# alibaba/EasyParallelLibrary

Measured on AMD Instinct MI355X. Metric: samples_per_sec, higher is better.
Workload: dtype bf16; 1 GPU; model=bert-large, global_batch=128, seq_len=512, parallelism=dp1

## Files before the change

csrc/bindings.hip:

```cpp

#include <hip/hip_runtime.h>
#include <torch/extension.h>
#include <ATen/hip/impl/HIPStreamMasqueradingAsCUDA.h>

#include <cstdint>

#include "kernels/attn_block_order.h"

namespace epl {
void register_comm(py::module& m);
}

extern "C" {
void epl_fused_adamw(float*, unsigned short*, const void*, bool, float*,
                     float*, int64_t, float, float, float, float, float, int,
                     float, hipStream_t);
void epl_lamb_phase1(const float*, const void*, bool, float*, float*, float*,
                     const int*, float*, float*, int64_t, float, float, float,
                     float, int, float, hipStream_t);
void epl_lamb_phase2(float*, unsigned short*, const float*, const int*,
                     const float*, int64_t, float, hipStream_t);
void epl_layer_norm_fwd(void*, const void*, const void*, void*, const void*,
                        const void*, float*, float*, int64_t, int64_t, float,
                        bool, hipStream_t);
void epl_layer_norm_bwd(void*, float*, float*, const void*, const void*,
                        const void*, const float*, const float*, float*,
                        float*, int64_t, int64_t, int64_t, bool,
                        hipStream_t);
void epl_layer_norm_bwd_fused(void*, float*, float*, float*, const void*,
                              const void*, const void*, const void*,
                              const float*, const float*, float*, float*,
                              float*, int64_t, int64_t, int64_t, bool,
                              hipStream_t);
void epl_bias_gelu_fwd(void*, const void*, const void*, int64_t, int64_t,
                       bool, hipStream_t);
void epl_bias_gelu_bwd(void*, float*, const void*, const void*, const void*,
                       float*, int64_t, int64_t, int64_t, bool,
                       hipStream_t);
void epl_ce_rowstats(const void*, const int64_t*, float*, float*, float*,
                     int64_t, int64_t, int64_t, int64_t, bool, hipStream_t);
void epl_ce_backward(void*, const void*, const int64_t*, const float*,
                     const float*, const float*, int64_t, int64_t, int64_t,
                     int64_t, float, bool, hipStream_t);
void epl_scale(void*, int64_t, float, bool, hipStream_t);
void epl_f32_to_bf16(unsigned short*, const float*, int64_t, hipStream_t);
void epl_bf16_to_f32(float*, const unsigned short*, int64_t, hipStream_t);
void epl_sqnorm(const void*, int64_t, float*, bool, hipStream_t);
void epl_colsum(void*, const void*, float*, int64_t, int64_t, int64_t,
                bool, hipStream_t);
void run_mfma_probe(const unsigned short*, const unsigned short*, float*,
                    hipStream_t);
void run_tr_read_probe(short*, short*, int, hipStream_t);
void run_block_order_probe(int*, int, int, hipStream_t);
void epl_moe_dispatch_fwd(void*, const void*, const int64_t*,
                          const int64_t*, const int64_t*, int64_t, int64_t,
                          int64_t, hipStream_t);
void epl_moe_dispatch_bwd(void*, const void*, const int64_t*,
                          const int64_t*, const int64_t*, int64_t, int64_t,
                          int64_t, int64_t, hipStream_t);
void epl_moe_combine_fwd(void*, const void*, const float*, const int64_t*,
                         const int64_t*, const int64_t*, int64_t, int64_t,
                         int64_t, int64_t, hipStream_t);
void epl_moe_combine_bwd(void*, float*, const void*, const void*,
                         const float*, const int64_t*, const int64_t*,
                         const int64_t*, int64_t, int64_t, int64_t,
                         hipStream_t);
int64_t epl_moe_router_waves(int64_t, int64_t);
void epl_moe_router_fwd(const void*, int64_t*, float*, float*, int64_t*,
                        float*, float*, float*, int*, int64_t, int64_t,
                        int64_t, bool, bool, hipStream_t);
void epl_moe_router_bwd(void*, const void*, const float*, const int64_t*,
                        const float*, const int64_t*, const float*,
                        const float*, int64_t, int64_t, int64_t, bool, bool,
                        hipStream_t);
void epl_attn_fwd(const void*, const void*, const void*, void*, float*,
                  int64_t, int64_t, float, bool, int64_t, int64_t,
                  const int64_t*,
                  const int64_t*, unsigned int*, int64_t,
                  unsigned long long, int, float, const int*, hipStream_t);
void epl_attn_bwd(const void*, const void*, const void*, const void*,
                  const void*, const float*, float*, void*, void*, void*,
                  int64_t, int64_t, float, bool, int64_t, const int64_t*,
                  const int64_t*, const int64_t*, const int64_t*, int,
                  const unsigned int*, int64_t, float, int64_t,
                  const float*, const int*, hipStream_t);
void epl_rms_norm_fwd(void*, const void*, const void*, void*, const void*,
                      float*, int64_t, int64_t, float, hipStream_t);
int64_t epl_rms_norm_bwd_parts(int64_t, int64_t);
void epl_rms_norm_bwd(void*, float*, const void*, const void*, const void*,
                      const float*, const void*, float*, int64_t, int64_t,
                      hipStream_t);
void epl_rope(void*, const float*, const float*, int64_t, int64_t, int64_t,
              int64_t, int64_t, int64_t, int64_t, int64_t, bool,
              hipStream_t);
void epl_swiglu_fwd(void*, const void*, int64_t, int64_t, hipStream_t);
void epl_swiglu_bwd(void*, const void*, const void*, int64_t, int64_t,
                    hipStream_t);
}

namespace {

hipStream_t cur_stream() {
  return c10::hip::getCurrentHIPStreamMasqueradingAsCUDA().stream();
}

void check(const at::Tensor& t, at::ScalarType dtype, const char* name) {
  TORCH_CHECK(t.is_cuda(), name, " must be a device tensor");
  TORCH_CHECK(t.is_contiguous(), name, " must be contiguous");
  TORCH_CHECK(t.scalar_type() == dtype, name, " has dtype ", t.scalar_type(),
              ", expected ", dtype);
}

void check_arena(const at::Tensor& t, const char* name) {
  TORCH_CHECK(t.is_cuda(), name, " must be a device tensor");
  TORCH_CHECK(t.is_contiguous(), name, " must be contiguous");
}

void check_aligned(const at::Tensor& t, size_t bytes, const char* name) {
  TORCH_CHECK(reinterpret_cast<uintptr_t>(t.data_ptr()) % bytes == 0, name,
              " must start on a ", bytes, "-byte boundary");
}

bool is_bf16(const at::Tensor& t) {
  TORCH_CHECK(t.scalar_type() == at::kBFloat16 || t.scalar_type() == at::kFloat,
              "expected bf16 or fp32, got ", t.scalar_type());
  return t.scalar_type() == at::kBFloat16;
}

void fused_adamw(at::Tensor master, c10::optional<at::Tensor> param_bf16,
                 at::Tensor grad, at::Tensor m, at::Tensor v, double lr,
                 double beta1, double beta2, double eps, double weight_decay,
                 int64_t step, double inv_scale) {
  check(master, at::kFloat, "master");
  check(m, at::kFloat, "m");
  check(v, at::kFloat, "v");
  check_arena(grad, "grad");
  const bool gbf = is_bf16(grad);
  unsigned short* pb = nullptr;
  if (param_bf16.has_value()) {
    check(*param_bf16, at::kBFloat16, "param_bf16");
    TORCH_CHECK(param_bf16->numel() == master.numel(),
                "arena size mismatch");
    check_aligned(*param_bf16, 16, "param_bf16");
    pb = reinterpret_cast<unsigned short*>(param_bf16->data_ptr());
  }
  const int64_t n = master.numel();
  TORCH_CHECK(grad.numel() == n && m.numel() == n && v.numel() == n,
              "arena size mismatch");
  check_aligned(master, 32, "master");
  check_aligned(m, 32, "m");
  check_aligned(v, 32, "v");
  check_aligned(grad, gbf ? 16 : 32, "grad");
  epl_fused_adamw(master.data_ptr<float>(), pb, grad.data_ptr(), gbf,
                  m.data_ptr<float>(), v.data_ptr<float>(), n, (float)lr,
                  (float)beta1, (float)beta2, (float)eps, (float)weight_decay,
                  (int)step, (float)inv_scale, cur_stream());
}

void lamb_phase1(at::Tensor master, at::Tensor grad, at::Tensor m,
                 at::Tensor v, at::Tensor update, at::Tensor chunk_of,
                 at::Tensor wnorm_sq, at::Tensor unorm_sq, double beta1,
                 double beta2, double eps, double weight_decay, int64_t step,
                 double inv_scale) {
  check(master, at::kFloat, "master");
  check(update, at::kFloat, "update");
  check(chunk_of, at::kInt, "chunk_of");
  const bool gbf = is_bf16(grad);
  epl_lamb_phase1(master.data_ptr<float>(), grad.data_ptr(), gbf,
                  m.data_ptr<float>(), v.data_ptr<float>(),
                  update.data_ptr<float>(), chunk_of.data_ptr<int>(),
                  wnorm_sq.data_ptr<float>(), unorm_sq.data_ptr<float>(),
                  master.numel(), (float)beta1, (float)beta2, (float)eps,
                  (float)weight_decay, (int)step, (float)inv_scale,
                  cur_stream());
}

void lamb_phase2(at::Tensor master, c10::optional<at::Tensor> param_bf16,
                 at::Tensor update, at::Tensor chunk_of, at::Tensor ratio,
                 double lr) {
  check(master, at::kFloat, "master");
  unsigned short* pb = nullptr;
  if (param_bf16.has_value())
    pb = reinterpret_cast<unsigned short*>(param_bf16->data_ptr());
  epl_lamb_phase2(master.data_ptr<float>(), pb, update.data_ptr<float>(),
                  chunk_of.data_ptr<int>(), ratio.data_ptr<float>(),
                  master.numel(), (float)lr, cur_stream());
}

void layer_norm_fwd(at::Tensor out, at::Tensor x,
                    c10::optional<at::Tensor> res,
                    c10::optional<at::Tensor> sum_out, at::Tensor gamma,
                    at::Tensor beta, at::Tensor mean, at::Tensor rstd,
                    double eps) {
  const bool bf16 = is_bf16(x);
  const int64_t cols = x.size(-1);
  const int64_t rows = x.numel() / cols;
  TORCH_CHECK(!bf16 || cols % 8 == 0, "bf16 LayerNorm needs cols % 8 == 0");
  check(mean, at::kFloat, "mean");
  check(rstd, at::kFloat, "rstd");
  const void* res_p = nullptr;
  void* sum_p = nullptr;
  if (res.has_value()) {
    TORCH_CHECK(sum_out.has_value(),
                "fused residual LayerNorm needs sum_out");
    TORCH_CHECK(res->numel() == x.numel() && sum_out->numel() == x.numel());
    res_p = res->data_ptr();
    sum_p = sum_out->data_ptr();
  }
  epl_layer_norm_fwd(out.data_ptr(), x.data_ptr(), res_p, sum_p,
                     gamma.data_ptr(), beta.data_ptr(),
                     mean.data_ptr<float>(), rstd.data_ptr<float>(), rows,
                     cols, (float)eps, bf16, cur_stream());
}

void layer_norm_bwd(at::Tensor dx, at::Tensor dgamma, at::Tensor dbeta,
                    at::Tensor dy, at::Tensor x, at::Tensor gamma,
                    at::Tensor mean, at::Tensor rstd) {
  const bool bf16 = is_bf16(x);
  const int64_t cols = x.size(-1);
  const int64_t rows = x.numel() / cols;
  TORCH_CHECK(!bf16 || cols % 8 == 0, "bf16 LayerNorm needs cols % 8 == 0");
  TORCH_CHECK((size_t)cols * 2 * sizeof(float) <= 128 * 1024,
              "LayerNorm backward supports cols <= 16384");
  check(dgamma, at::kFloat, "dgamma");
  check(dbeta, at::kFloat, "dbeta");
  float* dgp = nullptr;
  float* dbp = nullptr;
  at::Tensor ws;
  const bool fast = bf16 && cols % 8 == 0 && cols <= 2048;
  int64_t nparts = 0;
  if (fast) {
    const int64_t wave_rows = (rows + 3) / 4;
    nparts = (wave_rows < 1024 ? wave_rows : 1024) * 4;
    ws = at::empty({2, nparts, cols}, dgamma.options());
    dgp = ws.data_ptr<float>();
    dbp = dgp + nparts * cols;
  }
  epl_layer_norm_bwd(dx.data_ptr(), dgamma.data_ptr<float>(),
                     dbeta.data_ptr<float>(), dy.data_ptr(), x.data_ptr(),
                     gamma.data_ptr(), mean.data_ptr<float>(),
                     rstd.data_ptr<float>(), dgp, dbp, nparts, rows, cols,
                     bf16, cur_stream());
}

void layer_norm_bwd_fused(at::Tensor dx, at::Tensor dgamma, at::Tensor dbeta,
                          at::Tensor dy, at::Tensor x, at::Tensor gamma,
                          at::Tensor mean, at::Tensor rstd,
                          c10::optional<at::Tensor> dadd,
                          c10::optional<at::Tensor> colsum_out) {
  const bool bf16 = is_bf16(x);
  const int64_t cols = x.size(-1);
  const int64_t rows = x.numel() / cols;
  TORCH_CHECK(!bf16 || cols % 8 == 0, "bf16 LayerNorm needs cols % 8 == 0");
  TORCH_CHECK((size_t)cols * 2 * sizeof(float) <= 128 * 1024,
              "LayerNorm backward supports cols <= 16384");
  check(dgamma, at::kFloat, "dgamma");
  check(dbeta, at::kFloat, "dbeta");
  TORCH_CHECK(dx.numel() == x.numel() && dy.numel() == x.numel());
  TORCH_CHECK(dgamma.numel() == cols && dbeta.numel() == cols);
  const bool fast = bf16 && cols % 8 == 0 && cols <= 2048;
  const bool fused = dadd.has_value() || colsum_out.has_value();
  TORCH_CHECK(fast || !fused,
              "layer_norm_bwd_fused: dadd/colsum_out need the bf16 fast "
              "path (cols % 8 == 0, cols <= 2048)");
  const void* dadd_p = nullptr;
  float* cs_out = nullptr;
  if (dadd.has_value()) {
    check(*dadd, x.scalar_type(), "dadd");
    TORCH_CHECK(dadd->numel() == x.numel(), "dadd shape mismatch");
    dadd_p = dadd->data_ptr();
  }
  if (colsum_out.has_value()) {
    check(*colsum_out, at::kFloat, "colsum_out");
    TORCH_CHECK(colsum_out->numel() == cols, "colsum_out shape mismatch");
    cs_out = colsum_out->data_ptr<float>();
  }
  float* dgp = nullptr;
  float* dbp = nullptr;
  float* csp = nullptr;
  at::Tensor ws;
  int64_t nparts = 0;
  if (fast) {
    const int64_t wave_rows = (rows + 3) / 4;
    nparts = (wave_rows < 1024 ? wave_rows : 1024) * 4;
    ws = at::empty({cs_out ? 3 : 2, nparts, cols}, dgamma.options());
    dgp = ws.data_ptr<float>();
    dbp = dgp + nparts * cols;
    if (cs_out) csp = dbp + nparts * cols;
  }
  epl_layer_norm_bwd_fused(dx.data_ptr(), dgamma.data_ptr<float>(),
                           dbeta.data_ptr<float>(), cs_out, dy.data_ptr(),
                           x.data_ptr(), gamma.data_ptr(), dadd_p,
                           mean.data_ptr<float>(), rstd.data_ptr<float>(),
                           dgp, dbp, csp, nparts, rows, cols, bf16,
                           cur_stream());
}

void bias_gelu_fwd(at::Tensor out, at::Tensor x, at::Tensor bias) {
  const bool bf16 = is_bf16(x);
  const int64_t cols = x.size(-1);
  const int64_t rows = x.numel() / cols;
  TORCH_CHECK(!bf16 || cols % 8 == 0, "bf16 bias_gelu needs cols % 8 == 0");
  epl_bias_gelu_fwd(out.data_ptr(), x.data_ptr(), bias.data_ptr(), rows, cols,
                    bf16, cur_stream());
}

void bias_gelu_bwd(at::Tensor dx, at::Tensor dbias, at::Tensor dy,
                   at::Tensor x, at::Tensor bias) {
  const bool bf16 = is_bf16(x);
  const int64_t cols = x.size(-1);
  const int64_t rows = x.numel() / cols;
  TORCH_CHECK(!bf16 || cols % 8 == 0, "bf16 bias_gelu needs cols % 8 == 0");
  TORCH_CHECK((size_t)cols * sizeof(float) <= 128 * 1024,
              "bias_gelu backward supports cols <= 32768");
  check(dbias, at::kFloat, "dbias");
  float* dbp = nullptr;
  int64_t nwaves = 0;
  at::Tensor ws;
  if (bf16 && cols % 512 == 0) {
    const int64_t segs = cols / 512;
    int64_t per_seg = rows < 1024 ? rows : 1024;
    per_seg = (per_seg + 3) / 4 * 4;
    nwaves = segs * per_seg;
    ws = at::empty({nwaves, 512}, dbias.options());
    dbp = ws.data_ptr<float>();
  }
  epl_bias_gelu_bwd(dx.data_ptr(), dbias.data_ptr<float>(), dy.data_ptr(),
                    x.data_ptr(), bias.data_ptr(), dbp, nwaves, rows, cols,
                    bf16, cur_stream());
}

void ce_rowstats(at::Tensor logits, at::Tensor targets, at::Tensor row_max,
                 at::Tensor row_sumexp, at::Tensor target_logit,
                 int64_t vocab_begin, int64_t ignore_index) {
  const bool bf16 = is_bf16(logits);
  const int64_t cols = logits.size(-1);
  const int64_t rows = logits.numel() / cols;
  check(targets, at::kLong, "targets");
  epl_ce_rowstats(logits.data_ptr(), targets.data_ptr<int64_t>(),
                  row_max.data_ptr<float>(), row_sumexp.data_ptr<float>(),
                  target_logit.data_ptr<float>(), rows, cols, vocab_begin,
                  ignore_index, bf16, cur_stream());
}

void ce_backward(at::Tensor dlogits, at::Tensor logits, at::Tensor targets,
                 at::Tensor gmax, at::Tensor gsumexp, at::Tensor dloss,
                 int64_t vocab_begin, int64_t ignore_index, double scale) {
  const bool bf16 = is_bf16(logits);
  const int64_t cols = logits.size(-1);
  const int64_t rows = logits.numel() / cols;
  epl_ce_backward(dlogits.data_ptr(), logits.data_ptr(),
                  targets.data_ptr<int64_t>(), gmax.data_ptr<float>(),
                  gsumexp.data_ptr<float>(), dloss.data_ptr<float>(), rows,
                  cols, vocab_begin, ignore_index, (float)scale, bf16,
                  cur_stream());
}

void scale_(at::Tensor t, double s) {
  check_arena(t, "t");
  const bool bf16 = is_bf16(t);
  check_aligned(t, 16, "t");
  epl_scale(t.data_ptr(), t.numel(), (float)s, bf16, cur_stream());
}

void f32_to_bf16(at::Tensor dst, at::Tensor src) {
  check(dst, at::kBFloat16, "dst");
  check(src, at::kFloat, "src");
  TORCH_CHECK(dst.numel() == src.numel());
  check_aligned(dst, 16, "dst");
  check_aligned(src, 16, "src");
  epl_f32_to_bf16(reinterpret_cast<unsigned short*>(dst.data_ptr()),
                  src.data_ptr<float>(), src.numel(), cur_stream());
}

void bf16_to_f32(at::Tensor dst, at::Tensor src) {
  check(dst, at::kFloat, "dst");
  check(src, at::kBFloat16, "src");
  TORCH_CHECK(dst.numel() == src.numel());
  check_aligned(dst, 16, "dst");
  check_aligned(src, 16, "src");
  epl_bf16_to_f32(dst.data_ptr<float>(),
                  reinterpret_cast<unsigned short*>(src.data_ptr()),
                  src.numel(), cur_stream());
}

static void attn_strides(const at::Tensor& t, int64_t* out3,
                         const char* name) {
  TORCH_CHECK(t.dim() == 4 && (t.size(3) == 64 || t.size(3) == 128), name,
              " must be [B,H,S,64|128]");
  TORCH_CHECK(t.stride(3) == 1, name, " last dim must be contiguous");
  TORCH_CHECK(t.stride(2) % 8 == 0 && t.stride(1) % 8 == 0,
              name, " row strides must be 16-byte aligned");
  out3[0] = t.stride(0);
  out3[1] = t.stride(1);
  out3[2] = t.stride(2);
}

static void attn_check_grid(int64_t bh, int64_t seq, bool causal) {
  const int64_t nqb = (seq + 127) / 128;
  TORCH_CHECK(nqb <= 65535, "attention: seq ", seq, " needs ", nqb,
              " 128-row blocks, more than the 65535 a launch can hold");
  TORCH_CHECK(causal || bh <= 65535, "attention: non-causal batch*heads ",
              bh, " exceeds the 65535 blocks of gridDim.y");
}

static const int* attn_seqlens(const c10::optional<at::Tensor>& seqlens,
                               const at::Tensor& q) {
  if (!seqlens.has_value()) return nullptr;
  check(*seqlens, at::kInt, "seqlens");
  TORCH_CHECK(seqlens->numel() == q.size(0), "seqlens must hold ",
              q.size(0), " lengths (one per sample), got ",
              seqlens->numel());
  TORCH_CHECK(seqlens->device() == q.device(),
              "seqlens must be on the device of q");
  return seqlens->data_ptr<int>();
}

void attn_fwd(at::Tensor q, at::Tensor k, at::Tensor v, at::Tensor out,
              at::Tensor lse, double scale, bool causal,
              c10::optional<at::Tensor> drop_mask, int64_t seed,
              int64_t drop_thresh, double inv_keep,
              c10::optional<at::Tensor> seqlens) {
  TORCH_CHECK(q.is_cuda() && q.scalar_type() == at::kBFloat16);
  int64_t in_s[3], o_s[3], tmp[3];
  attn_strides(q, in_s, "q");
  attn_strides(k, tmp, "k");
  TORCH_CHECK(tmp[0] == in_s[0] && tmp[1] == in_s[1] && tmp[2] == in_s[2],
              "q/k/v must share strides");
  attn_strides(v, tmp, "v");
  TORCH_CHECK(tmp[0] == in_s[0] && tmp[1] == in_s[1] && tmp[2] == in_s[2],
              "q/k/v must share strides");
  attn_strides(out, o_s, "out");
  check(lse, at::kFloat, "lse");
  const int64_t heads = q.size(1);
  const int64_t seq = q.size(2);
  const int64_t head_dim = q.size(3);
  const int64_t bh = q.size(0) * heads;
  attn_check_grid(bh, seq, causal);
  unsigned int* mptr = nullptr;
  int64_t mask_w = (seq + 31) / 32;
  if (drop_mask.has_value()) {
    check(*drop_mask, at::kInt, "drop_mask");
    TORCH_CHECK(drop_mask->numel() == bh * seq * mask_w,
                "drop_mask size mismatch");
    TORCH_CHECK(drop_thresh > 0 && drop_thresh < 256, "drop_thresh range");
    mptr = reinterpret_cast<unsigned int*>(drop_mask->data_ptr());
  }
  epl_attn_fwd(q.data_ptr(), k.data_ptr(), v.data_ptr(), out.data_ptr(),
               lse.data_ptr<float>(), bh, seq, (float)scale, causal, heads,
               head_dim, in_s, o_s, mptr, mask_w,
               (unsigned long long)seed, (int)drop_thresh,
               (float)inv_keep, attn_seqlens(seqlens, q), cur_stream());
}

void attn_bwd(at::Tensor q, at::Tensor k, at::Tensor v, at::Tensor out,
              at::Tensor dout, at::Tensor lse, at::Tensor delta_ws,
              at::Tensor dq, at::Tensor dk, at::Tensor dv, double scale,
              bool causal, bool split_dkdv,
              c10::optional<at::Tensor> drop_mask, double inv_keep,
              c10::optional<at::Tensor> dlse,
              c10::optional<at::Tensor> seqlens) {
  int64_t in_s[3], o_s[3], do_s[3], g_s[3], tmp[3];
  attn_strides(q, in_s, "q");
  attn_strides(out, o_s, "out");
  attn_strides(dout, do_s, "dout");
  attn_strides(dq, g_s, "dq");
  attn_strides(dk, tmp, "dk");
  TORCH_CHECK(tmp[0] == g_s[0] && tmp[1] == g_s[1] && tmp[2] == g_s[2],
              "dq/dk/dv must share strides");
  attn_strides(dv, tmp, "dv");
  TORCH_CHECK(tmp[0] == g_s[0] && tmp[1] == g_s[1] && tmp[2] == g_s[2],
              "dq/dk/dv must share strides");
  const int64_t heads = q.size(1);
  const int64_t seq = q.size(2);
  const int64_t bh = q.size(0) * heads;
  attn_check_grid(bh, seq, causal);
  check(delta_ws, at::kFloat, "delta_ws");
  const unsigned int* mptr = nullptr;
  int64_t mask_w = (seq + 31) / 32;
  if (drop_mask.has_value()) {
    check(*drop_mask, at::kInt, "drop_mask");
    mptr = reinterpret_cast<const unsigned int*>(drop_mask->data_ptr());
  }
  const float* dlse_ptr = nullptr;
  if (dlse.has_value()) {
    check(*dlse, at::kFloat, "dlse");
    TORCH_CHECK(dlse->numel() == bh * seq, "dlse size mismatch");
    dlse_ptr = dlse->data_ptr<float>();
  }
  epl_attn_bwd(q.data_ptr(), k.data_ptr(), v.data_ptr(), out.data_ptr(),
               dout.data_ptr(), lse.data_ptr<float>(),
               delta_ws.data_ptr<float>(), dq.data_ptr(), dk.data_ptr(),
               dv.data_ptr(), bh, seq, (float)scale, causal, heads, in_s,
               o_s, do_s, g_s, split_dkdv ? 1 : 0, mptr, mask_w,
               (float)inv_keep, q.size(3), dlse_ptr,
               attn_seqlens(seqlens, q), cur_stream());
}

void tr_read_probe(at::Tensor out_gather, at::Tensor out_tr,
                   int64_t head_dim) {
  TORCH_CHECK(head_dim == 64 || head_dim == 128, "head_dim must be 64|128");
  check(out_gather, at::kShort, "out_gather");
  check(out_tr, at::kShort, "out_tr");
  const int64_t n = 4 * (head_dim / 32) * 64 * 8;
  TORCH_CHECK(out_gather.numel() == n && out_tr.numel() == n,
              "probe outputs must hold ", n, " elements");
  run_tr_read_probe(reinterpret_cast<short*>(out_gather.data_ptr()),
                    reinterpret_cast<short*>(out_tr.data_ptr()),
                    (int)head_dim, cur_stream());
}

void attn_block_order_probe(at::Tensor out, int64_t n, int64_t bh) {
  check(out, at::kInt, "out");
  TORCH_CHECK(n >= 1 && n <= 65535 && bh >= 1 && bh <= 65535,
              "grid dimensions must lie in [1, 65535]");
  TORCH_CHECK(out.numel() == 2 * n * bh, "out must hold ", 2 * n * bh,
              " elements");
  run_block_order_probe(out.data_ptr<int>(), (int)n, (int)bh, cur_stream());
}

at::Tensor attn_block_order_host(int64_t n, int64_t bh) {
  TORCH_CHECK(n >= 1 && n <= 65535 && bh >= 1 && bh <= 65535,
              "grid dimensions must lie in [1, 65535]");
  at::Tensor out = at::empty({n * bh, 2}, at::kInt);
  int* p = out.data_ptr<int>();
  for (int64_t y = 0; y < bh; ++y)
    for (int64_t x = 0; x < n; ++x) {
      const attn_order::Block b = attn_order::block_of(
          (unsigned)x, (unsigned)y, (unsigned)n, (unsigned)bh);
      p[2 * (x + n * y)] = (int)b.bh;
      p[2 * (x + n * y) + 1] = (int)b.blk;
    }
  return out;
}

void mfma_probe(at::Tensor A, at::Tensor B, at::Tensor D) {
  check(A, at::kBFloat16, "A");
  check(B, at::kBFloat16, "B");
  check(D, at::kFloat, "D");
  run_mfma_probe(reinterpret_cast<const unsigned short*>(A.data_ptr()),
                 reinterpret_cast<const unsigned short*>(B.data_ptr()),
                 D.data_ptr<float>(), cur_stream());
}

static void check_idx(const at::Tensor& t, const char* name) {
  TORCH_CHECK(t.is_cuda() && t.is_contiguous() &&
              t.scalar_type() == at::kLong, name,
              " must be a contiguous int64 device tensor");
}

void moe_dispatch_fwd(at::Tensor disp, at::Tensor x, at::Tensor fe,
                      at::Tensor pos, at::Tensor ft, int64_t cap) {
  check(disp, at::kBFloat16, "disp");
  check(x, at::kBFloat16, "x");
  check_idx(fe, "fe"); check_idx(pos, "pos"); check_idx(ft, "ft");
  const int64_t hidden = x.size(-1);
  TORCH_CHECK(hidden % 8 == 0, "hidden % 8");
  epl_moe_dispatch_fwd(disp.data_ptr(), x.data_ptr(),
                       fe.data_ptr<int64_t>(), pos.data_ptr<int64_t>(),
                       ft.data_ptr<int64_t>(), fe.numel(), hidden, cap,
                       cur_stream());
}

void moe_dispatch_bwd(at::Tensor dx, at::Tensor ddisp, at::Tensor fe,
                      at::Tensor pos, at::Tensor inv, int64_t k,
                      int64_t cap) {
  check(dx, at::kBFloat16, "dx");
  check(ddisp, at::kBFloat16, "ddisp");
  check_idx(fe, "fe"); check_idx(pos, "pos"); check_idx(inv, "inv");
  const int64_t hidden = dx.size(-1);
  epl_moe_dispatch_bwd(dx.data_ptr(), ddisp.data_ptr(),
                       fe.data_ptr<int64_t>(), pos.data_ptr<int64_t>(),
                       inv.data_ptr<int64_t>(), dx.numel() / hidden, k,
                       hidden, cap, cur_stream());
}

void moe_combine_fwd(at::Tensor out, at::Tensor h, at::Tensor fw,
                     at::Tensor fe, at::Tensor pos, at::Tensor inv,
                     int64_t k, int64_t cap) {
  check(out, at::kBFloat16, "out");
  check(h, at::kBFloat16, "h");
  check(fw, at::kFloat, "fw");
  check_idx(fe, "fe"); check_idx(pos, "pos"); check_idx(inv, "inv");
  const int64_t hidden = out.size(-1);
  epl_moe_combine_fwd(out.data_ptr(), h.data_ptr(), fw.data_ptr<float>(),
                      fe.data_ptr<int64_t>(), pos.data_ptr<int64_t>(),
                      inv.data_ptr<int64_t>(), out.numel() / hidden, k,
                      hidden, cap, cur_stream());
}

void moe_combine_bwd(at::Tensor dh, at::Tensor dfw, at::Tensor dout,
                     at::Tensor h, at::Tensor fw, at::Tensor fe,
                     at::Tensor pos, at::Tensor ft, int64_t cap) {
  check(dh, at::kBFloat16, "dh");
  check(dout, at::kBFloat16, "dout");
  check(h, at::kBFloat16, "h");
  check(fw, at::kFloat, "fw");
  check(dfw, at::kFloat, "dfw");
  check_idx(fe, "fe"); check_idx(pos, "pos"); check_idx(ft, "ft");
  const int64_t hidden = dh.size(-1);
  epl_moe_combine_bwd(dh.data_ptr(), dfw.data_ptr<float>(),
                      dout.data_ptr(), h.data_ptr(), fw.data_ptr<float>(),
                      fe.data_ptr<int64_t>(), pos.data_ptr<int64_t>(),
                      ft.data_ptr<int64_t>(), fe.numel(), hidden, cap,
                      cur_stream());
}

static bool aligned16(const at::Tensor& t) {
  return reinterpret_cast<uintptr_t>(t.data_ptr()) % 16 == 0;
}

static void router_extents(const at::Tensor& logits, int64_t k, int64_t* n,
                           int64_t* e) {
  TORCH_CHECK(logits.is_cuda() && logits.is_contiguous() &&
              logits.dim() == 2,
              "logits must be a contiguous 2-D device tensor");
  *n = logits.size(0);
  *e = logits.size(1);
  TORCH_CHECK(k == 1 || k == 2, "moe router: k must be 1 or 2, got ", k);
  TORCH_CHECK(*e >= 2 && *e <= 256,
              "moe router: 2 <= num_experts <= 256, got ", *e);
  TORCH_CHECK(*n >= 1 && *n < (int64_t(1) << 30),
              "moe router: 1 <= tokens < 2^30, got ", *n);
}

void moe_router_fwd(at::Tensor logits, int64_t k, at::Tensor topi,
                    at::Tensor topw, at::Tensor lse, at::Tensor counts,
                    at::Tensor psum, at::Tensor losses) {
  const bool bf16 = is_bf16(logits);
  int64_t n, e;
  router_extents(logits, k, &n, &e);
  check_idx(topi, "topi");
  check(topw, at::kFloat, "topw");
  check(lse, at::kFloat, "lse");
  check_idx(counts, "counts");
  check(psum, at::kFloat, "psum");
  check(losses, at::kFloat, "losses");
  TORCH_CHECK(topi.numel() == n * k && topw.numel() == n * k,
              "topi / topw must hold tokens * k elements");
  TORCH_CHECK(lse.numel() == n, "lse must hold one element per token");
  TORCH_CHECK(counts.numel() == e && psum.numel() == e,
              "counts / psum must hold one element per expert");
  TORCH_CHECK(losses.numel() == 2, "losses must hold 2 elements");
  const int64_t waves = epl_moe_router_waves(n, e);
  at::Tensor p_part = at::empty({waves * e + waves},
                                logits.options().dtype(at::kFloat));
  at::Tensor c_part = at::empty({waves * e},
                                logits.options().dtype(at::kInt));
  epl_moe_router_fwd(logits.data_ptr(), topi.data_ptr<int64_t>(),
                     topw.data_ptr<float>(), lse.data_ptr<float>(),
                     counts.data_ptr<int64_t>(), psum.data_ptr<float>(),
                     losses.data_ptr<float>(), p_part.data_ptr<float>(),
                     c_part.data_ptr<int>(), n, e, k, bf16,
                     aligned16(logits), cur_stream());
}

void moe_router_bwd(at::Tensor dlogits, at::Tensor logits, at::Tensor lse,
                    at::Tensor topi, at::Tensor dw, at::Tensor counts,
                    at::Tensor g_bal, at::Tensor g_z, int64_t k) {
  const bool bf16 = is_bf16(logits);
  int64_t n, e;
  router_extents(logits, k, &n, &e);
  check(dlogits, logits.scalar_type(), "dlogits");
  TORCH_CHECK(dlogits.numel() == n * e, "dlogits must match logits");
  check(lse, at::kFloat, "lse");
  check_idx(topi, "topi");
  check(dw, at::kFloat, "dw");
  check_idx(counts, "counts");
  check(g_bal, at::kFloat, "g_bal");
  check(g_z, at::kFloat, "g_z");
  TORCH_CHECK(lse.numel() == n, "lse must hold one element per token");
  TORCH_CHECK(topi.numel() == n * k && dw.numel() == n * k,
              "topi / dw must hold tokens * k elements");
  TORCH_CHECK(counts.numel() == e,
              "counts must hold one element per expert");
  TORCH_CHECK(g_bal.numel() == 1 && g_z.numel() == 1,
              "g_bal / g_z must hold one element");
  epl_moe_router_bwd(dlogits.data_ptr(), logits.data_ptr(),
                     lse.data_ptr<float>(), topi.data_ptr<int64_t>(),
                     dw.data_ptr<float>(), counts.data_ptr<int64_t>(),
                     g_bal.data_ptr<float>(), g_z.data_ptr<float>(), n, e, k,
                     bf16, aligned16(logits) && aligned16(dlogits),
                     cur_stream());
}

void colsum(at::Tensor dy, at::Tensor db, at::Tensor partial) {
  const bool bf16 = is_bf16(dy);
  TORCH_CHECK(dy.is_cuda() && dy.is_contiguous() && dy.dim() == 2,
              "dy must be a contiguous 2-D device tensor");
  const int64_t rows = dy.size(0), cols = dy.size(1);
  TORCH_CHECK(cols % 8 == 0, "cols must be a multiple of 8");
  TORCH_CHECK(db.numel() == cols && db.scalar_type() == dy.scalar_type());
  const int64_t stripes = partial.numel() / cols;
  TORCH_CHECK(stripes >= 1 && partial.scalar_type() == at::kFloat);
  epl_colsum(db.data_ptr(), dy.data_ptr(), partial.data_ptr<float>(), rows,
             cols, stripes, bf16, cur_stream());
}

void sqnorm(at::Tensor t, at::Tensor out) {
  check_arena(t, "t");
  const bool bf16 = is_bf16(t);
  check(out, at::kFloat, "out");
  TORCH_CHECK(out.numel() >= 1, "out must hold one element");
  epl_sqnorm(t.data_ptr(), t.numel(), out.data_ptr<float>(), bf16,
             cur_stream());
}


static void check_llama_bf16(const at::Tensor& t, const at::Device& dev,
                             const char* name) {
  check(t, at::kBFloat16, name);
  TORCH_CHECK(t.device() == dev, name, " is on another device");
  TORCH_CHECK(aligned16(t), name, " must be 16-byte aligned");
}

static void check_llama_f32(const at::Tensor& t, const at::Device& dev,
                            int64_t numel, const char* name) {
  check(t, at::kFloat, name);
  TORCH_CHECK(t.device() == dev, name, " is on another device");
  TORCH_CHECK(aligned16(t), name, " must be 16-byte aligned");
  TORCH_CHECK(t.numel() == numel, name, " must hold ", numel, " elements");
}

static void rms_extents(const at::Tensor& x, int64_t* rows, int64_t* cols) {
  TORCH_CHECK(x.dim() >= 1 && x.numel() > 0, "rms_norm: empty input");
  *cols = x.size(-1);
  *rows = x.numel() / *cols;
  TORCH_CHECK(*cols % 8 == 0 && *cols >= 8 && *cols <= 8192,
              "rms_norm: native widths are multiples of 8 up to 8192, got ",
              *cols);
}

void rms_norm_fwd(at::Tensor out, at::Tensor x, c10::optional<at::Tensor> res,
                  c10::optional<at::Tensor> s_out, at::Tensor gamma,
                  at::Tensor rstd, double eps) {
  int64_t rows, cols;
  const at::Device dev = x.device();
  check_llama_bf16(x, dev, "x");
  rms_extents(x, &rows, &cols);
  check_llama_bf16(out, dev, "out");
  check_llama_bf16(gamma, dev, "gamma");
  TORCH_CHECK(out.numel() == x.numel(), "out must match x");
  TORCH_CHECK(gamma.numel() == cols, "gamma must hold cols elements");
  check_llama_f32(rstd, dev, rows, "rstd");
  TORCH_CHECK(res.has_value() == s_out.has_value(),
              "rms_norm_fwd: res and s come together");
  const void* res_p = nullptr;
  void* s_p = nullptr;
  if (res.has_value()) {
    check_llama_bf16(*res, dev, "res");
    check_llama_bf16(*s_out, dev, "s");
    TORCH_CHECK(res->numel() == x.numel() && s_out->numel() == x.numel(),
                "res and s must match x");
    res_p = res->data_ptr();
    s_p = s_out->data_ptr();
  }
  epl_rms_norm_fwd(out.data_ptr(), x.data_ptr(), res_p, s_p,
                   gamma.data_ptr(), rstd.data_ptr<float>(), rows, cols,
                   (float)eps, cur_stream());
}

void rms_norm_bwd(at::Tensor dx, at::Tensor dgamma, at::Tensor dy,
                  at::Tensor s, at::Tensor gamma, at::Tensor rstd,
                  c10::optional<at::Tensor> dadd) {
  int64_t rows, cols;
  const at::Device dev = s.device();
  check_llama_bf16(s, dev, "s");
  rms_extents(s, &rows, &cols);
  check_llama_bf16(dx, dev, "dx");
  check_llama_bf16(dy, dev, "dy");
  check_llama_bf16(gamma, dev, "gamma");
  TORCH_CHECK(dx.numel() == s.numel() && dy.numel() == s.numel(),
              "dx and dy must match s");
  TORCH_CHECK(gamma.numel() == cols, "gamma must hold cols elements");
  check_llama_f32(dgamma, dev, cols, "dgamma");
  check_llama_f32(rstd, dev, rows, "rstd");
  const void* dadd_p = nullptr;
  if (dadd.has_value()) {
    check_llama_bf16(*dadd, dev, "dadd");
    TORCH_CHECK(dadd->numel() == s.numel(), "dadd must match s");
    dadd_p = dadd->data_ptr();
  }
  const int64_t nparts = epl_rms_norm_bwd_parts(rows, cols);
  at::Tensor ws = at::empty({nparts, cols}, dgamma.options());
  epl_rms_norm_bwd(dx.data_ptr(), dgamma.data_ptr<float>(), dy.data_ptr(),
                   s.data_ptr(), gamma.data_ptr(), rstd.data_ptr<float>(),
                   dadd_p, ws.data_ptr<float>(), rows, cols, cur_stream());
}

void rope_(at::Tensor x, at::Tensor cos_t, at::Tensor sin_t, int64_t pos0,
           bool inverse) {
  TORCH_CHECK(x.is_cuda() && x.scalar_type() == at::kBFloat16,
              "rope_: x must be a bf16 device tensor");
  TORCH_CHECK(x.dim() == 4, "rope_: x must be a [B, S, N, D] view");
  const int64_t b = x.size(0), s = x.size(1), n = x.size(2), d = x.size(3);
  TORCH_CHECK(d == 64 || d == 128, "rope_: head_dim must be 64 or 128, got ",
              d);
  TORCH_CHECK(x.stride(3) == 1, "rope_: last dim must be contiguous");
  for (int i = 0; i < 3; ++i)
    TORCH_CHECK(x.size(i) == 1 || (x.stride(i) % 8 == 0 && x.stride(i) >= d),
                "rope_: stride ", i, " must be a multiple of 8 elements "
                "and at least one head, got ", x.stride(i));
  TORCH_CHECK(aligned16(x), "rope_: x must be 16-byte aligned");
  TORCH_CHECK(b * s * n * (d / 16) < (int64_t(1) << 31),
              "rope_: too many elements for one launch");
  const at::Device dev = x.device();
  TORCH_CHECK(cos_t.dim() == 2 && cos_t.size(1) == d / 2,
              "rope_: tables must be [L, D / 2]");
  check_llama_f32(cos_t, dev, cos_t.size(0) * (d / 2), "cos");
  check_llama_f32(sin_t, dev, cos_t.numel(), "sin");
  TORCH_CHECK(pos0 >= 0 && pos0 + s <= cos_t.size(0), "rope_: positions ",
              pos0, " .. ", pos0 + s, " exceed the table length ",
              cos_t.size(0));
  epl_rope(x.data_ptr(), cos_t.data_ptr<float>(), sin_t.data_ptr<float>(),
           x.stride(0), x.stride(1), x.stride(2), b, s, n, d, pos0, inverse,
           cur_stream());
}

static void swiglu_extents(const at::Tensor& gu, int64_t* rows, int64_t* f) {
  TORCH_CHECK(gu.dim() >= 1 && gu.numel() > 0, "swiglu: empty input");
  TORCH_CHECK(gu.size(-1) % 16 == 0, "swiglu: the packed width 2F needs "
              "F % 8 == 0, got ", gu.size(-1));
  *f = gu.size(-1) / 2;
  *rows = gu.numel() / gu.size(-1);
  TORCH_CHECK(*f <= (int64_t(1) << 21), "swiglu: F too large");
}

void swiglu_fwd(at::Tensor out, at::Tensor gu) {
  int64_t rows, f;
  const at::Device dev = gu.device();
  check_llama_bf16(gu, dev, "gu");
  swiglu_extents(gu, &rows, &f);
  check_llama_bf16(out, dev, "out");
  TORCH_CHECK(out.numel() == rows * f, "out must be [rows, F]");
  epl_swiglu_fwd(out.data_ptr(), gu.data_ptr(), rows, f, cur_stream());
}

void swiglu_bwd(at::Tensor dgu, at::Tensor dy, at::Tensor gu) {
  int64_t rows, f;
  const at::Device dev = gu.device();
  check_llama_bf16(gu, dev, "gu");
  swiglu_extents(gu, &rows, &f);
  check_llama_bf16(dgu, dev, "dgu");
  check_llama_bf16(dy, dev, "dy");
  TORCH_CHECK(dgu.numel() == gu.numel(), "dgu must match gu");
  TORCH_CHECK(dy.numel() == rows * f, "dy must be [rows, F]");
  epl_swiglu_bwd(dgu.data_ptr(), dy.data_ptr(), gu.data_ptr(), rows, f,
                 cur_stream());
}

}

PYBIND11_MODULE(TORCH_EXTENSION_NAME, m) {
  m.doc() = "MI355X-native parallel library: RCCL comm core + CDNA4 kernels";
  epl::register_comm(m);
  m.def("fused_adamw", &fused_adamw);
  m.def("colsum", &colsum);
  m.def("lamb_phase1", &lamb_phase1);
  m.def("lamb_phase2", &lamb_phase2);
  m.def("layer_norm_fwd", &layer_norm_fwd);
  m.def("layer_norm_bwd", &layer_norm_bwd);
  m.def("layer_norm_bwd_fused", &layer_norm_bwd_fused, py::arg("dx"),
        py::arg("dgamma"), py::arg("dbeta"), py::arg("dy"), py::arg("x"),
        py::arg("gamma"), py::arg("mean"), py::arg("rstd"),
        py::arg("dadd") = py::none(), py::arg("colsum_out") = py::none());
  m.def("bias_gelu_fwd", &bias_gelu_fwd);
  m.def("bias_gelu_bwd", &bias_gelu_bwd);
  m.def("ce_rowstats", &ce_rowstats);
  m.def("ce_backward", &ce_backward);
  m.def("scale_", &scale_);
  m.def("f32_to_bf16", &f32_to_bf16);
  m.def("bf16_to_f32", &bf16_to_f32);
  m.def("sqnorm", &sqnorm);
  m.def("mfma_probe", &mfma_probe);
  m.def("tr_read_probe", &tr_read_probe);
  m.def("attn_block_order_probe", &attn_block_order_probe);
  m.def("attn_block_order_host", &attn_block_order_host);
  m.def("moe_dispatch_fwd", &moe_dispatch_fwd);
  m.def("moe_dispatch_bwd", &moe_dispatch_bwd);
  m.def("moe_combine_fwd", &moe_combine_fwd);
  m.def("moe_combine_bwd", &moe_combine_bwd);
  m.def("moe_router_fwd", &moe_router_fwd);
  m.def("moe_router_bwd", &moe_router_bwd);
  m.def("moe_router_waves", [](int64_t n, int64_t e) {
    return epl_moe_router_waves(n, e);
  });
  m.def("attn_fwd", &attn_fwd, py::arg("q"), py::arg("k"), py::arg("v"),
        py::arg("out"), py::arg("lse"), py::arg("scale"), py::arg("causal"),
        py::arg("drop_mask"), py::arg("seed"), py::arg("drop_thresh"),
        py::arg("inv_keep"), py::arg("seqlens") = py::none());
  m.def("attn_bwd", &attn_bwd, py::arg("q"), py::arg("k"), py::arg("v"),
        py::arg("out"), py::arg("dout"), py::arg("lse"),
        py::arg("delta_ws"), py::arg("dq"), py::arg("dk"), py::arg("dv"),
        py::arg("scale"), py::arg("causal"), py::arg("split_dkdv"),
        py::arg("drop_mask"), py::arg("inv_keep"), py::arg("dlse"),
        py::arg("seqlens") = py::none());
  m.def("rms_norm_fwd", &rms_norm_fwd, py::arg("out"), py::arg("x"),
        py::arg("res"), py::arg("s"), py::arg("gamma"), py::arg("rstd"),
        py::arg("eps"));
  m.def("rms_norm_bwd", &rms_norm_bwd, py::arg("dx"), py::arg("dgamma"),
        py::arg("dy"), py::arg("s"), py::arg("gamma"), py::arg("rstd"),
        py::arg("dadd") = py::none());
  m.def("rope_", &rope_, py::arg("x"), py::arg("cos"), py::arg("sin"),
        py::arg("pos0"), py::arg("inverse"));
  m.def("swiglu_fwd", &swiglu_fwd);
  m.def("swiglu_bwd", &swiglu_bwd);
}
```

csrc/kernels/kernels.hip:

```cpp

#include <hip/hip_runtime.h>
#include <hip/hip_bf16.h>
#include <cstdint>
#include <cmath>

#define DEV __device__ __forceinline__

namespace {

constexpr int kBlock = 256;
constexpr int kMaxGrid = 4096;

DEV float bf2f(unsigned short u) {
  unsigned int x = (unsigned int)u << 16;
  return __uint_as_float(x);
}

using f32x2 = __attribute__((ext_vector_type(2))) float;
using bf16v2 = __attribute__((ext_vector_type(2))) __bf16;

DEV unsigned int cvt_pk_bf16(float a, float b) {
  f32x2 f = {a, b};
  return __builtin_bit_cast(unsigned int, __builtin_convertvector(f, bf16v2));
}

DEV unsigned short f2bf(float f) {
  return (unsigned short)cvt_pk_bf16(f, f);
}

struct ushort8 {
  unsigned short v[8];
};
struct float8 {
  float v[8];
};

DEV float8 load_bf16x8(const unsigned short* p) {
  const ushort8 raw = *reinterpret_cast<const ushort8*>(p);
  float8 f;
#pragma unroll
  for (int i = 0; i < 8; ++i) f.v[i] = bf2f(raw.v[i]);
  return f;
}

DEV void store_bf16x8(unsigned short* p, const float8& f) {
  *reinterpret_cast<uint4*>(p) =
      make_uint4(cvt_pk_bf16(f.v[0], f.v[1]), cvt_pk_bf16(f.v[2], f.v[3]),
                 cvt_pk_bf16(f.v[4], f.v[5]), cvt_pk_bf16(f.v[6], f.v[7]));
}

DEV float8 load_f32x8(const float* p) {
  float8 f;
  const float4 a = *reinterpret_cast<const float4*>(p);
  const float4 b = *reinterpret_cast<const float4*>(p + 4);
  f.v[0] = a.x; f.v[1] = a.y; f.v[2] = a.z; f.v[3] = a.w;
  f.v[4] = b.x; f.v[5] = b.y; f.v[6] = b.z; f.v[7] = b.w;
  return f;
}

DEV void store_f32x8(float* p, const float8& f) {
  *reinterpret_cast<float4*>(p) = make_float4(f.v[0], f.v[1], f.v[2], f.v[3]);
  *reinterpret_cast<float4*>(p + 4) =
      make_float4(f.v[4], f.v[5], f.v[6], f.v[7]);
}

inline int grid_for(int64_t work_items) {
  int64_t blocks = (work_items + kBlock - 1) / kBlock;
  return (int)(blocks < kMaxGrid ? (blocks > 0 ? blocks : 1) : kMaxGrid);
}

inline float inv_bias_correction(float beta, int step) {
  return (float)(1.0 / (1.0 - std::pow((double)beta, (double)step)));
}

DEV float block_reduce_sum(float val, float* lds ) {
#pragma unroll
  for (int off = 32; off > 0; off >>= 1)
    val += __shfl_down(val, off, 64);
  const int wave = threadIdx.x >> 6;
  const int lane = threadIdx.x & 63;
  const int nwaves = blockDim.x >> 6;
  if (lane == 0) lds[wave] = val;
  __syncthreads();
  if (wave == 0) {
    val = lane < nwaves ? lds[lane] : 0.f;
#pragma unroll
    for (int off = 2; off > 0; off >>= 1)
      val += __shfl_down(val, off, 64);
    if (lane == 0) lds[0] = val;
  }
  __syncthreads();
  return lds[0];
}

DEV float block_reduce_max(float val, float* lds) {
#pragma unroll
  for (int off = 32; off > 0; off >>= 1)
    val = fmaxf(val, __shfl_down(val, off, 64));
  const int wave = threadIdx.x >> 6;
  const int lane = threadIdx.x & 63;
  const int nwaves = blockDim.x >> 6;
  if (lane == 0) lds[wave] = val;
  __syncthreads();
  if (wave == 0) {
    val = lane < nwaves ? lds[lane] : -INFINITY;
#pragma unroll
    for (int off = 2; off > 0; off >>= 1)
      val = fmaxf(val, __shfl_down(val, off, 64));
    if (lane == 0) lds[0] = val;
  }
  __syncthreads();
  return lds[0];
}

template <bool GRAD_BF16, bool HAS_BF16_PARAM>
__global__ void fused_adamw_kernel(
    float* __restrict__ master, unsigned short* __restrict__ param,
    const void* __restrict__ grad_raw, float* __restrict__ m,
    float* __restrict__ v, int64_t n, float lr, float beta1, float beta2,
    float eps, float weight_decay, float inv_bias1, float inv_bias2,
    float inv_scale) {
  const int64_t nvec = n / 8;
  for (int64_t i = blockIdx.x * blockDim.x + threadIdx.x; i < nvec;
       i += (int64_t)gridDim.x * blockDim.x) {
    const int64_t base = i * 8;
    float8 g;
    if (GRAD_BF16)
      g = load_bf16x8(
          reinterpret_cast<const unsigned short*>(grad_raw) + base);
    else
      g = load_f32x8(reinterpret_cast<const float*>(grad_raw) + base);
    float8 pm = load_f32x8(master + base);
    float8 mm = load_f32x8(m + base);
    float8 vv = load_f32x8(v + base);
#pragma unroll
    for (int k = 0; k < 8; ++k) {
      float gk = g.v[k] * inv_scale;
      float mk = beta1 * mm.v[k] + (1.f - beta1) * gk;
      float vk = beta2 * vv.v[k] + (1.f - beta2) * gk * gk;
      float mhat = mk * inv_bias1;
      float vhat = vk * inv_bias2;
      float pk = pm.v[k];
      pk -= lr * (mhat / (sqrtf(vhat) + eps) + weight_decay * pk);
      mm.v[k] = mk;
      vv.v[k] = vk;
      pm.v[k] = pk;
    }
    store_f32x8(m + base, mm);
    store_f32x8(v + base, vv);
    store_f32x8(master + base, pm);
    if (HAS_BF16_PARAM) store_bf16x8(param + base, pm);
  }
  const int64_t tail = nvec * 8;
  for (int64_t i = tail + blockIdx.x * blockDim.x + threadIdx.x; i < n;
       i += (int64_t)gridDim.x * blockDim.x) {
    float gk = (GRAD_BF16
                    ? bf2f(reinterpret_cast<const unsigned short*>(grad_raw)[i])
                    : reinterpret_cast<const float*>(grad_raw)[i]) *
               inv_scale;
    float mk = beta1 * m[i] + (1.f - beta1) * gk;
    float vk = beta2 * v[i] + (1.f - beta2) * gk * gk;
    float pk = master[i];
    pk -= lr * ((mk * inv_bias1) / (sqrtf(vk * inv_bias2) + eps) +
                weight_decay * pk);
    m[i] = mk;
    v[i] = vk;
    master[i] = pk;
    if (HAS_BF16_PARAM) param[i] = f2bf(pk);
  }
}

__global__ void lamb_phase1_kernel(
    const float* __restrict__ master, const void* __restrict__ grad_raw,
    bool grad_bf16, float* __restrict__ m, float* __restrict__ v,
    float* __restrict__ update, const int* __restrict__ chunk_of,
    float* __restrict__ wnorm_sq, float* __restrict__ unorm_sq, int64_t n,
    float beta1, float beta2, float eps, float weight_decay, float inv_bias1,
    float inv_bias2, float inv_scale) {
  for (int64_t i = blockIdx.x * blockDim.x + threadIdx.x; i < n;
       i += (int64_t)gridDim.x * blockDim.x) {
    float gk = (grad_bf16
                    ? bf2f(reinterpret_cast<const unsigned short*>(grad_raw)[i])
                    : reinterpret_cast<const float*>(grad_raw)[i]) *
               inv_scale;
    float mk = beta1 * m[i] + (1.f - beta1) * gk;
    float vk = beta2 * v[i] + (1.f - beta2) * gk * gk;
    m[i] = mk;
    v[i] = vk;
    float pk = master[i];
    float u = (mk * inv_bias1) / (sqrtf(vk * inv_bias2) + eps) +
              weight_decay * pk;
    update[i] = u;
    const int c = chunk_of[i >> 3];
    atomicAdd(&wnorm_sq[c], pk * pk);
    atomicAdd(&unorm_sq[c], u * u);
  }
}

__global__ void lamb_phase2_kernel(float* __restrict__ master,
                                   unsigned short* __restrict__ param,
                                   const float* __restrict__ update,
                                   const int* __restrict__ chunk_of,
                                   const float* __restrict__ ratio, int64_t n,
                                   float lr) {
  for (int64_t i = blockIdx.x * blockDim.x + threadIdx.x; i < n;
       i += (int64_t)gridDim.x * blockDim.x) {
    const int c = chunk_of[i >> 3];
    float pk = master[i] - lr * ratio[c] * update[i];
    master[i] = pk;
    if (param != nullptr) param[i] = f2bf(pk);
  }
}

template <bool HAS_RES, int CHUNKS>
__global__ void layer_norm_fwd_bf16_kernel(
    void* __restrict__ out, const void* __restrict__ x,
    const void* __restrict__ res, void* __restrict__ sum_out,
    const void* __restrict__ gamma, const void* __restrict__ beta,
    float* __restrict__ mean_out, float* __restrict__ rstd_out, int64_t rows,
    int64_t cols, float eps) {
  __shared__ float lds[8];
  using T = unsigned short;
  float8 cache[CHUNKS];
  float8 gw[CHUNKS], bw[CHUNKS];
#pragma unroll
  for (int k = 0; k < CHUNKS; ++k) {
    const int64_t c = ((int64_t)threadIdx.x + k * blockDim.x) * 8;
    if (c < cols) {
      gw[k] = load_bf16x8(reinterpret_cast<const T*>(gamma) + c);
      bw[k] = load_bf16x8(reinterpret_cast<const T*>(beta) + c);
    }
  }
  for (int64_t row = blockIdx.x; row < rows; row += gridDim.x) {
    const int64_t base = row * cols;
    float piv = bf2f(reinterpret_cast<const T*>(x)[base]);
    if (HAS_RES) piv += bf2f(reinterpret_cast<const T*>(res)[base]);
    float sum = 0.f;
#pragma unroll
    for (int k = 0; k < CHUNKS; ++k) {
      const int64_t c = ((int64_t)threadIdx.x + k * blockDim.x) * 8;
      if (c >= cols) continue;
      float8 f = load_bf16x8(reinterpret_cast<const T*>(x) + base + c);
      if (HAS_RES) {
        float8 r = load_bf16x8(reinterpret_cast<const T*>(res) + base + c);
#pragma unroll
        for (int j = 0; j < 8; ++j) f.v[j] += r.v[j];
        store_bf16x8(reinterpret_cast<T*>(sum_out) + base + c, f);
      }
      cache[k] = f;
#pragma unroll
      for (int j = 0; j < 8; ++j) sum += f.v[j] - piv;
    }
    sum = block_reduce_sum(sum, lds);
    const float mean = piv + sum / cols;
    float ssq = 0.f;
#pragma unroll
    for (int k = 0; k < CHUNKS; ++k) {
      const int64_t c = ((int64_t)threadIdx.x + k * blockDim.x) * 8;
      if (c >= cols) continue;
#pragma unroll
      for (int j = 0; j < 8; ++j) {
        const float d = cache[k].v[j] - mean;
        ssq += d * d;
      }
    }
    __syncthreads();
    ssq = block_reduce_sum(ssq, lds);
    const float rstd = rsqrtf(ssq / cols + eps);
    if (threadIdx.x == 0) {
      mean_out[row] = mean;
      rstd_out[row] = rstd;
    }
#pragma unroll
    for (int k = 0; k < CHUNKS; ++k) {
      const int64_t c = ((int64_t)threadIdx.x + k * blockDim.x) * 8;
      if (c >= cols) continue;
      float8 y;
#pragma unroll
      for (int j = 0; j < 8; ++j)
        y.v[j] = (cache[k].v[j] - mean) * rstd * gw[k].v[j] + bw[k].v[j];
      store_bf16x8(reinterpret_cast<T*>(out) + base + c, y);
    }
    __syncthreads();
  }
}

template <bool BF16, bool HAS_RES>
__global__ void layer_norm_fwd_kernel(
    void* __restrict__ out, const void* __restrict__ x,
    const void* __restrict__ res, void* __restrict__ sum_out,
    const void* __restrict__ gamma, const void* __restrict__ beta,
    float* __restrict__ mean_out, float* __restrict__ rstd_out, int64_t rows,
    int64_t cols, float eps) {
  __shared__ float lds[8];
  using T = unsigned short;
  for (int64_t row = blockIdx.x; row < rows; row += gridDim.x) {
    const int64_t base = row * cols;
    auto s_at = [&](int64_t i) -> float {
      float fv = BF16 ? bf2f(reinterpret_cast<const T*>(x)[i])
                      : reinterpret_cast<const float*>(x)[i];
      if (HAS_RES)
        fv += BF16 ? bf2f(reinterpret_cast<const T*>(res)[i])
                   : reinterpret_cast<const float*>(res)[i];
      return fv;
    };
    const float piv = s_at(base);
    float sum = 0.f;
    for (int64_t c = threadIdx.x; c < cols; c += blockDim.x) {
      const float fv = s_at(base + c);
      if (HAS_RES) {
        if (BF16)
          reinterpret_cast<T*>(sum_out)[base + c] = f2bf(fv);
        else
          reinterpret_cast<float*>(sum_out)[base + c] = fv;
      }
      sum += fv - piv;
    }
    sum = block_reduce_sum(sum, lds);
    const float mean = piv + sum / cols;
    float ssq = 0.f;
    for (int64_t c = threadIdx.x; c < cols; c += blockDim.x) {
      const float d = s_at(base + c) - mean;
      ssq += d * d;
    }
    __syncthreads();
    ssq = block_reduce_sum(ssq, lds);
    const float rstd = rsqrtf(ssq / cols + eps);
    if (threadIdx.x == 0) {
      mean_out[row] = mean;
      rstd_out[row] = rstd;
    }
    const void* nin = HAS_RES ? sum_out : x;
    for (int64_t c = threadIdx.x; c < cols; c += blockDim.x) {
      float fv = BF16 ? bf2f(reinterpret_cast<const T*>(nin)[base + c])
                      : reinterpret_cast<const float*>(nin)[base + c];
      float gv = BF16 ? bf2f(reinterpret_cast<const T*>(gamma)[c])
                      : reinterpret_cast<const float*>(gamma)[c];
      float bv = BF16 ? bf2f(reinterpret_cast<const T*>(beta)[c])
                      : reinterpret_cast<const float*>(beta)[c];
      float y = (fv - mean) * rstd * gv + bv;
      if (BF16)
        reinterpret_cast<T*>(out)[base + c] = f2bf(y);
      else
        reinterpret_cast<float*>(out)[base + c] = y;
    }
    __syncthreads();
  }
}

template <int CHUNKS, bool CACHE, bool DADD, bool COLSUM>
__global__ __launch_bounds__(256, CHUNKS == 1 ? 5 : 3) void
layer_norm_bwd_bf16_kernel(
    void* __restrict__ dx, float* __restrict__ dg_part,
    float* __restrict__ db_part, float* __restrict__ cs_part,
    const void* __restrict__ dy, const void* __restrict__ x,
    const void* __restrict__ gamma, const void* __restrict__ dadd,
    const float* __restrict__ mean_in, const float* __restrict__ rstd_in,
    int64_t rows, int64_t cols) {
  using T = unsigned short;
  const int lane = threadIdx.x & 63;
  const int wid = threadIdx.x >> 6;
  const int wpb = blockDim.x >> 6;
  constexpr bool FUSED = DADD || COLSUM;
  constexpr bool G_LDS = FUSED && CHUNKS == 4;
  constexpr bool G_PK = FUSED && CHUNKS == 1;
  constexpr bool G_F32 = !G_LDS && !G_PK;
  __shared__ __attribute__((aligned(16))) T g_lds[G_LDS ? CHUNKS * 512 : 8];
  float8 gw[G_F32 ? CHUNKS : 1], acc_dg[CHUNKS], acc_db[CHUNKS];
  uint4 gpk[G_PK ? CHUNKS : 1];
  float8 acc_cs[COLSUM ? CHUNKS : 1];
  if (G_LDS) {
    for (int64_t c = (int64_t)threadIdx.x * 8; c < cols;
         c += (int64_t)blockDim.x * 8)
      *reinterpret_cast<uint4*>(g_lds + c) =
          *reinterpret_cast<const uint4*>(reinterpret_cast<const T*>(gamma) +
                                          c);
    __syncthreads();
  }
  auto gamma_at = [&](int k, int64_t c) -> float8 {
    if (G_LDS) return load_bf16x8(g_lds + c);
    if (G_PK) {
      asm volatile("" : "+v"(gpk[k].x), "+v"(gpk[k].y), "+v"(gpk[k].z),
                   "+v"(gpk[k].w));
      return load_bf16x8(reinterpret_cast<const T*>(&gpk[k]));
    }
    return gw[k];
  };
#pragma unroll
  for (int k = 0; k < CHUNKS; ++k) {
    const int64_t c = ((int64_t)lane + k * 64) * 8;
#pragma unroll
    for (int j = 0; j < 8; ++j) {
      acc_dg[k].v[j] = 0.f;
      acc_db[k].v[j] = 0.f;
      if (COLSUM) acc_cs[k].v[j] = 0.f;
    }
    if (c < cols) {
      if (G_F32)
        gw[k] = load_bf16x8(reinterpret_cast<const T*>(gamma) + c);
      if (G_PK)
        gpk[k] = *reinterpret_cast<const uint4*>(
            reinterpret_cast<const T*>(gamma) + c);
    }
  }
  for (int64_t row = (int64_t)blockIdx.x * wpb + wid; row < rows;
       row += (int64_t)gridDim.x * wpb) {
    const int64_t base = row * cols;
    const float mean = mean_in[row];
    const float rstd = rstd_in[row];
    float sum_dyg = 0.f, sum_dygx = 0.f;
    float8 c_xhat[CACHE ? CHUNKS : 1], c_dy[CACHE ? CHUNKS : 1];
#pragma unroll
    for (int k = 0; k < CHUNKS; ++k) {
      const int64_t c = ((int64_t)lane + k * 64) * 8;
      if (c >= cols) continue;
      float8 d = load_bf16x8(reinterpret_cast<const T*>(dy) + base + c);
      float8 f = load_bf16x8(reinterpret_cast<const T*>(x) + base + c);
      const float8 g = gamma_at(k, c);
#pragma unroll
      for (int j = 0; j < 8; ++j) {
        const float xhat = (f.v[j] - mean) * rstd;
        const float dyg = d.v[j] * g.v[j];
        if (CACHE) {
          c_xhat[k].v[j] = xhat;
          c_dy[k].v[j] = d.v[j];
        }
        sum_dyg += dyg;
        sum_dygx += dyg * xhat;
      }
    }
#pragma unroll
    for (int off = 32; off > 0; off >>= 1) {
      sum_dyg += __shfl_down(sum_dyg, off, 64);
      sum_dygx += __shfl_down(sum_dygx, off, 64);
    }
    sum_dyg = __shfl(sum_dyg, 0, 64);
    sum_dygx = __shfl(sum_dygx, 0, 64);
    const float inv_cols = 1.f / cols;
#pragma unroll
    for (int k = 0; k < CHUNKS; ++k) {
      const int64_t c = ((int64_t)lane + k * 64) * 8;
      if (c >= cols) continue;
      float8 dv, xh;
      if (CACHE) {
        dv = c_dy[k];
        xh = c_xhat[k];
      } else {
        float8 d = load_bf16x8(reinterpret_cast<const T*>(dy) + base + c);
        float8 f = load_bf16x8(reinterpret_cast<const T*>(x) + base + c);
#pragma unroll
        for (int j = 0; j < 8; ++j) {
          dv.v[j] = d.v[j];
          xh.v[j] = (f.v[j] - mean) * rstd;
        }
      }
      const float8 g = gamma_at(k, c);
      float8 o;
#pragma unroll
      for (int j = 0; j < 8; ++j) {
        const float dyg = dv.v[j] * g.v[j];
        o.v[j] = (dyg - (sum_dyg + xh.v[j] * sum_dygx) * inv_cols) * rstd;
        acc_dg[k].v[j] += dv.v[j] * xh.v[j];
        acc_db[k].v[j] += dv.v[j];
      }
      if (DADD) {
        const float8 a =
            load_bf16x8(reinterpret_cast<const T*>(dadd) + base + c);
#pragma unroll
        for (int j = 0; j < 8; ++j) o.v[j] += a.v[j];
      }
      if (COLSUM) {
#pragma unroll
        for (int j = 0; j < 8; ++j) acc_cs[k].v[j] += o.v[j];
      }
      store_bf16x8(reinterpret_cast<T*>(dx) + base + c, o);
    }
  }
  const int64_t prow = ((int64_t)blockIdx.x * wpb + wid) * cols;
#pragma unroll
  for (int k = 0; k < CHUNKS; ++k) {
    const int64_t c = ((int64_t)lane + k * 64) * 8;
    if (c >= cols) continue;
    store_f32x8(dg_part + prow + c, acc_dg[k]);
    store_f32x8(db_part + prow + c, acc_db[k]);
    if (COLSUM) store_f32x8(cs_part + prow + c, acc_cs[k]);
  }
}

template <bool COLSUM>
__global__ void ln_bwd_partial_reduce_kernel(
    float* __restrict__ dgamma, float* __restrict__ dbeta,
    float* __restrict__ colsum, const float* __restrict__ dg_part,
    const float* __restrict__ db_part, const float* __restrict__ cs_part,
    int64_t nparts, int64_t cols) {
  const int64_t c = (int64_t)blockIdx.x * blockDim.x + threadIdx.x;
  if (c >= cols) return;
  float sg = 0.f, sb = 0.f, sc = 0.f;
  for (int64_t p = blockIdx.y; p < nparts; p += gridDim.y) {
    sg += dg_part[p * cols + c];
    sb += db_part[p * cols + c];
    if (COLSUM) sc += cs_part[p * cols + c];
  }
  atomicAdd(&dgamma[c], sg);
  atomicAdd(&dbeta[c], sb);
  if (COLSUM) atomicAdd(&colsum[c], sc);
}

template <bool BF16>
__global__ void layer_norm_bwd_kernel(
    void* __restrict__ dx, float* __restrict__ dgamma,
    float* __restrict__ dbeta, const void* __restrict__ dy,
    const void* __restrict__ x, const void* __restrict__ gamma,
    const float* __restrict__ mean_in, const float* __restrict__ rstd_in,
    int64_t rows, int64_t cols) {
  extern __shared__ __attribute__((aligned(16))) char smem[];
  float* part_dg = reinterpret_cast<float*>(smem);
  float* part_db = part_dg + cols;
  __shared__ float lds[8];
  using T = unsigned short;
  for (int64_t c = threadIdx.x; c < cols; c += blockDim.x) {
    part_dg[c] = 0.f;
    part_db[c] = 0.f;
  }
  __syncthreads();
  for (int64_t row = blockIdx.x; row < rows; row += gridDim.x) {
    const int64_t base = row * cols;
    const float mean = mean_in[row];
    const float rstd = rstd_in[row];
    float sum_dyg = 0.f, sum_dygx = 0.f;
    for (int64_t c = threadIdx.x; c < cols; c += blockDim.x) {
      const float dv = BF16 ? bf2f(reinterpret_cast<const T*>(dy)[base + c])
                            : reinterpret_cast<const float*>(dy)[base + c];
      const float fv = BF16 ? bf2f(reinterpret_cast<const T*>(x)[base + c])
                            : reinterpret_cast<const float*>(x)[base + c];
      const float gv = BF16 ? bf2f(reinterpret_cast<const T*>(gamma)[c])
                            : reinterpret_cast<const float*>(gamma)[c];
      const float xhat = (fv - mean) * rstd;
      const float dyg = dv * gv;
      sum_dyg += dyg;
      sum_dygx += dyg * xhat;
      part_dg[c] += dv * xhat;
      part_db[c] += dv;
    }
    __syncthreads();
    sum_dyg = block_reduce_sum(sum_dyg, lds);
    __syncthreads();
    sum_dygx = block_reduce_sum(sum_dygx, lds);
    const float inv_cols = 1.f / cols;
    for (int64_t c = threadIdx.x; c < cols; c += blockDim.x) {
      const float dv = BF16 ? bf2f(reinterpret_cast<const T*>(dy)[base + c])
                            : reinterpret_cast<const float*>(dy)[base + c];
      const float fv = BF16 ? bf2f(reinterpret_cast<const T*>(x)[base + c])
                            : reinterpret_cast<const float*>(x)[base + c];
      const float gv = BF16 ? bf2f(reinterpret_cast<const T*>(gamma)[c])
                            : reinterpret_cast<const float*>(gamma)[c];
      const float xhat = (fv - mean) * rstd;
      const float o = (dv * gv - (sum_dyg + xhat * sum_dygx) * inv_cols) *
                      rstd;
      if (BF16)
        reinterpret_cast<T*>(dx)[base + c] = f2bf(o);
      else
        reinterpret_cast<float*>(dx)[base + c] = o;
    }
    __syncthreads();
  }
  for (int64_t c = threadIdx.x; c < cols; c += blockDim.x) {
    atomicAdd(&dgamma[c], part_dg[c]);
    atomicAdd(&dbeta[c], part_db[c]);
  }
}

DEV float fast_tanh(float u) {
  return 1.f - 2.f / (__expf(2.f * u) + 1.f);
}

DEV float gelu_f(float x) {
  const float k0 = 0.7978845608028654f;
  const float k1 = 0.044715f;
  return 0.5f * x * (1.f + fast_tanh(k0 * (x + k1 * x * x * x)));
}

DEV float gelu_grad_f(float x) {
  const float k0 = 0.7978845608028654f;
  const float k1 = 0.044715f;
  const float t = fast_tanh(k0 * (x + k1 * x * x * x));
  const float dt = (1.f - t * t) * k0 * (1.f + 3.f * k1 * x * x);
  return 0.5f * (1.f + t) + 0.5f * x * dt;
}

DEV float gelu_sigmoid(float x) {
  constexpr float c0 = (float)(-2.0 * 0.7978845608028654 *
                               1.4426950408889634);
  constexpr float c1 = (float)(-2.0 * 0.7978845608028654 *
                               1.4426950408889634 * 0.044715);
  const float e = __builtin_amdgcn_exp2f(x * (c0 + c1 * x * x));
  return __builtin_amdgcn_rcpf(1.f + e);
}

DEV float gelu_lean(float x) { return x * gelu_sigmoid(x); }

DEV float gelu_grad_lean(float x) {
  constexpr float d0 = (float)(2.0 * 0.7978845608028654);
  constexpr float d1 = (float)(6.0 * 0.7978845608028654 * 0.044715);
  const float s = gelu_sigmoid(x);
  return s + x * s * (1.f - s) * (d0 + d1 * x * x);
}

DEV void store_bf16x8_pk(unsigned short* p, const float8& f) {
  *reinterpret_cast<uint4*>(p) =
      make_uint4(cvt_pk_bf16(f.v[0], f.v[1]), cvt_pk_bf16(f.v[2], f.v[3]),
                 cvt_pk_bf16(f.v[4], f.v[5]), cvt_pk_bf16(f.v[6], f.v[7]));
}

template <bool BF16>
__global__ void bias_gelu_fwd_kernel(void* __restrict__ out,
                                     const void* __restrict__ x,
                                     const void* __restrict__ bias,
                                     int64_t rows, int64_t cols) {
  using T = unsigned short;
  const int64_t n = rows * cols;
  if (BF16) {
    const unsigned vpr = (unsigned)(cols / 8);
    const unsigned g = blockIdx.x * blockDim.x + threadIdx.x;
    const unsigned rpp = (gridDim.x * blockDim.x) / vpr;
    const unsigned r0 = g / vpr;
    if (r0 >= rpp) return;
    const int64_t c = (int64_t)(g - r0 * vpr) * 8;
    const float8 b = load_bf16x8(reinterpret_cast<const T*>(bias) + c);
    for (int64_t row = r0; row < rows; row += rpp) {
      const int64_t base = row * cols + c;
      float8 f = load_bf16x8(reinterpret_cast<const T*>(x) + base);
      float8 o;
#pragma unroll
      for (int k = 0; k < 8; ++k) o.v[k] = gelu_lean(f.v[k] + b.v[k]);
      store_bf16x8_pk(reinterpret_cast<T*>(out) + base, o);
    }
  } else {
    for (int64_t i = blockIdx.x * blockDim.x + threadIdx.x; i < n;
         i += (int64_t)gridDim.x * blockDim.x) {
      const float xv = reinterpret_cast<const float*>(x)[i] +
                       reinterpret_cast<const float*>(bias)[i % cols];
      reinterpret_cast<float*>(out)[i] = gelu_f(xv);
    }
  }
}

__global__ void bias_gelu_bwd_bf16_kernel(
    void* __restrict__ dx, float* __restrict__ db_part,
    const void* __restrict__ dy, const void* __restrict__ x,
    const void* __restrict__ bias, int64_t rows, int64_t cols) {
  using T = unsigned short;
  const int lane = threadIdx.x & 63;
  const int wid = threadIdx.x >> 6;
  const int wpb = blockDim.x >> 6;
  const int64_t segs = cols / 512;
  const int64_t total = rows * segs;
  float8 acc;
#pragma unroll
  for (int j = 0; j < 8; ++j) acc.v[j] = 0.f;
  const int64_t wave_id = (int64_t)blockIdx.x * wpb + wid;
  const int64_t nwaves = (int64_t)gridDim.x * wpb;
  const int64_t myseg = wave_id % segs;
  const int64_t c0 = myseg * 512 + (int64_t)lane * 8;
  float8 bw = load_bf16x8(reinterpret_cast<const T*>(bias) + c0);
  for (int64_t row = wave_id / segs; row < rows; row += nwaves / segs) {
    const int64_t base = row * cols + c0;
    float8 d = load_bf16x8(reinterpret_cast<const T*>(dy) + base);
    float8 f = load_bf16x8(reinterpret_cast<const T*>(x) + base);
    float8 o;
#pragma unroll
    for (int j = 0; j < 8; ++j) {
      const float g = d.v[j] * gelu_grad_lean(f.v[j] + bw.v[j]);
      o.v[j] = g;
      acc.v[j] += g;
    }
    store_bf16x8_pk(reinterpret_cast<T*>(dx) + base, o);
  }
  store_f32x8(db_part + wave_id * 512 + (int64_t)lane * 8, acc);
}

__global__ void bias_gelu_db_reduce_kernel(
    float* __restrict__ dbias, const float* __restrict__ db_part,
    int64_t nwaves, int64_t segs) {
  const int64_t c = (int64_t)blockIdx.x * blockDim.x + threadIdx.x;
  if (c >= segs * 512) return;
  const int64_t seg = c / 512;
  const int64_t off = c % 512;
  float sum = 0.f;
  for (int64_t p = seg + blockIdx.y * segs; p < nwaves;
       p += (int64_t)gridDim.y * segs) {
    sum += db_part[p * 512 + off];
  }
  atomicAdd(&dbias[c], sum);
}

template <bool BF16>
__global__ void bias_gelu_bwd_kernel(void* __restrict__ dx,
                                     float* __restrict__ dbias,
                                     const void* __restrict__ dy,
                                     const void* __restrict__ x,
                                     const void* __restrict__ bias,
                                     int64_t rows, int64_t cols) {
  extern __shared__ __attribute__((aligned(16))) char smem[];
  float* part_db = reinterpret_cast<float*>(smem);
  using T = unsigned short;
  for (int64_t c = threadIdx.x; c < cols; c += blockDim.x) part_db[c] = 0.f;
  __syncthreads();
  for (int64_t row = blockIdx.x; row < rows; row += gridDim.x) {
    const int64_t base = row * cols;
    if (BF16) {
      for (int64_t c = threadIdx.x * 8; c < cols; c += (int64_t)blockDim.x * 8) {
        float8 d = load_bf16x8(reinterpret_cast<const T*>(dy) + base + c);
        float8 f = load_bf16x8(reinterpret_cast<const T*>(x) + base + c);
        float8 b = load_bf16x8(reinterpret_cast<const T*>(bias) + c);
        float8 o;
#pragma unroll
        for (int k = 0; k < 8; ++k) {
          const float g = d.v[k] * gelu_grad_f(f.v[k] + b.v[k]);
          o.v[k] = g;
          part_db[c + k] += g;
        }
        store_bf16x8(reinterpret_cast<T*>(dx) + base + c, o);
      }
    } else {
      for (int64_t c = threadIdx.x; c < cols; c += blockDim.x) {
        const float g = reinterpret_cast<const float*>(dy)[base + c] *
                        gelu_grad_f(reinterpret_cast<const float*>(x)[base + c] +
                                    reinterpret_cast<const float*>(bias)[c]);
        reinterpret_cast<float*>(dx)[base + c] = g;
        part_db[c] += g;
      }
    }
  }
  __syncthreads();
  for (int64_t c = threadIdx.x; c < cols; c += blockDim.x)
    atomicAdd(&dbias[c], part_db[c]);
}

template <bool BF16>
__global__ void ce_rowstats_kernel(const void* __restrict__ logits,
                                   const int64_t* __restrict__ targets,
                                   float* __restrict__ row_max,
                                   float* __restrict__ row_sumexp,
                                   float* __restrict__ target_logit,
                                   int64_t rows, int64_t cols,
                                   int64_t vocab_begin, int64_t ignore_index) {
  __shared__ float lds[8];
  using T = unsigned short;
  const bool vec = BF16 && (cols % 8 == 0);
  for (int64_t row = blockIdx.x; row < rows; row += gridDim.x) {
    const int64_t base = row * cols;
    float vmax = -INFINITY;
    if (vec) {
      const T* lr = reinterpret_cast<const T*>(logits) + base;
      for (int64_t c = threadIdx.x * 8; c < cols;
           c += (int64_t)blockDim.x * 8) {
        float8 f = load_bf16x8(lr + c);
#pragma unroll
        for (int k = 0; k < 8; ++k) vmax = fmaxf(vmax, f.v[k]);
      }
    } else {
      for (int64_t c = threadIdx.x; c < cols; c += blockDim.x) {
        const float v = BF16
            ? bf2f(reinterpret_cast<const T*>(logits)[base + c])
            : reinterpret_cast<const float*>(logits)[base + c];
        vmax = fmaxf(vmax, v);
      }
    }
    vmax = block_reduce_max(vmax, lds);
    __syncthreads();
    float sum = 0.f;
    if (vec) {
      const T* lr = reinterpret_cast<const T*>(logits) + base;
      for (int64_t c = threadIdx.x * 8; c < cols;
           c += (int64_t)blockDim.x * 8) {
        float8 f = load_bf16x8(lr + c);
#pragma unroll
        for (int k = 0; k < 8; ++k) sum += expf(f.v[k] - vmax);
      }
    } else {
      for (int64_t c = threadIdx.x; c < cols; c += blockDim.x) {
        const float v = BF16
            ? bf2f(reinterpret_cast<const T*>(logits)[base + c])
            : reinterpret_cast<const float*>(logits)[base + c];
        sum += expf(v - vmax);
      }
    }
    sum = block_reduce_sum(sum, lds);
    if (threadIdx.x == 0) {
      row_max[row] = vmax;
      row_sumexp[row] = sum;
      const int64_t tgt = targets[row];
      float tl = 0.f;
      if (tgt != ignore_index && tgt >= vocab_begin &&
          tgt < vocab_begin + cols) {
        const int64_t c = tgt - vocab_begin;
        tl = BF16 ? bf2f(reinterpret_cast<const T*>(logits)[base + c])
                  : reinterpret_cast<const float*>(logits)[base + c];
      }
      target_logit[row] = tl;
    }
    __syncthreads();
  }
}

template <bool BF16>
__global__ void ce_backward_kernel(void* __restrict__ dlogits,
                                   const void* __restrict__ logits,
                                   const int64_t* __restrict__ targets,
                                   const float* __restrict__ gmax,
                                   const float* __restrict__ gsumexp,
                                   const float* __restrict__ dloss,
                                   int64_t rows, int64_t cols,
                                   int64_t vocab_begin, int64_t ignore_index,
                                   float scale) {
  using T = unsigned short;
  const bool vec = BF16 && (cols % 8 == 0);
  for (int64_t row = blockIdx.x; row < rows; row += gridDim.x) {
    const int64_t base = row * cols;
    const float m = gmax[row];
    const float inv_sum = 1.f / gsumexp[row];
    const int64_t tgt = targets[row];
    const float dl = (tgt == ignore_index ? 0.f : dloss[row] * scale);
    const int64_t tc = tgt - vocab_begin;
    if (vec) {
      const T* lr = reinterpret_cast<const T*>(logits) + base;
      T* dr = reinterpret_cast<T*>(dlogits) + base;
      for (int64_t c = threadIdx.x * 8; c < cols;
           c += (int64_t)blockDim.x * 8) {
        float8 f = load_bf16x8(lr + c);
        float8 o;
#pragma unroll
        for (int k = 0; k < 8; ++k) {
          float g = expf(f.v[k] - m) * inv_sum;
          if (tc == c + k) g -= 1.f;
          o.v[k] = g * dl;
        }
        store_bf16x8(dr + c, o);
      }
    } else {
      for (int64_t c = threadIdx.x; c < cols; c += blockDim.x) {
        const float v = BF16
            ? bf2f(reinterpret_cast<const T*>(logits)[base + c])
            : reinterpret_cast<const float*>(logits)[base + c];
        float g = expf(v - m) * inv_sum;
        if (tc == c) g -= 1.f;
        g *= dl;
        if (BF16)
          reinterpret_cast<T*>(dlogits)[base + c] = f2bf(g);
        else
          reinterpret_cast<float*>(dlogits)[base + c] = g;
      }
    }
  }
}

__global__ void scale_f32_kernel(float* __restrict__ p, int64_t n, float s) {
  const int64_t nvec = n / 4;
  float4* p4 = reinterpret_cast<float4*>(p);
  for (int64_t i = blockIdx.x * blockDim.x + threadIdx.x; i < nvec;
       i += (int64_t)gridDim.x * blockDim.x) {
    float4 v = p4[i];
    v.x *= s; v.y *= s; v.z *= s; v.w *= s;
    p4[i] = v;
  }
  for (int64_t i = nvec * 4 + blockIdx.x * blockDim.x + threadIdx.x; i < n;
       i += (int64_t)gridDim.x * blockDim.x)
    p[i] *= s;
}

__global__ void scale_bf16_kernel(unsigned short* __restrict__ p, int64_t n,
                                  float s) {
  const int64_t nvec = n / 8;
  for (int64_t i = blockIdx.x * blockDim.x + threadIdx.x; i < nvec;
       i += (int64_t)gridDim.x * blockDim.x) {
    float8 v = load_bf16x8(p + i * 8);
#pragma unroll
    for (int k = 0; k < 8; ++k) v.v[k] *= s;
    store_bf16x8(p + i * 8, v);
  }
  for (int64_t i = nvec * 8 + blockIdx.x * blockDim.x + threadIdx.x; i < n;
       i += (int64_t)gridDim.x * blockDim.x)
    p[i] = f2bf(bf2f(p[i]) * s);
}

__global__ void f32_to_bf16_kernel(unsigned short* __restrict__ dst,
                                   const float* __restrict__ src, int64_t n) {
  const int64_t nvec = n / 8;
  for (int64_t i = blockIdx.x * blockDim.x + threadIdx.x; i < nvec;
       i += (int64_t)gridDim.x * blockDim.x)
    store_bf16x8(dst + i * 8, load_f32x8(src + i * 8));
  for (int64_t i = nvec * 8 + blockIdx.x * blockDim.x + threadIdx.x; i < n;
       i += (int64_t)gridDim.x * blockDim.x)
    dst[i] = f2bf(src[i]);
}

__global__ void bf16_to_f32_kernel(float* __restrict__ dst,
                                   const unsigned short* __restrict__ src,
                                   int64_t n) {
  const int64_t nvec = n / 8;
  for (int64_t i = blockIdx.x * blockDim.x + threadIdx.x; i < nvec;
       i += (int64_t)gridDim.x * blockDim.x)
    store_f32x8(dst + i * 8, load_bf16x8(src + i * 8));
  for (int64_t i = nvec * 8 + blockIdx.x * blockDim.x + threadIdx.x; i < n;
       i += (int64_t)gridDim.x * blockDim.x)
    dst[i] = bf2f(src[i]);
}

template <bool BF16>
__global__ void sqnorm_kernel(const void* __restrict__ p, int64_t n,
                              float* __restrict__ out) {
  __shared__ float lds[8];
  using T = unsigned short;
  float acc = 0.f;
  for (int64_t i = blockIdx.x * blockDim.x + threadIdx.x; i < n;
       i += (int64_t)gridDim.x * blockDim.x) {
    const float v = BF16 ? bf2f(reinterpret_cast<const T*>(p)[i])
                         : reinterpret_cast<const float*>(p)[i];
    acc += v * v;
  }
  acc = block_reduce_sum(acc, lds);
  if (threadIdx.x == 0) atomicAdd(out, acc);
}

}


template <bool BF16>
__global__ void colsum_partial_kernel(const void* __restrict__ dy,
                                      float* __restrict__ partial,
                                      int64_t rows, int64_t cols,
                                      int64_t stripes) {
  const int64_t c = ((int64_t)blockIdx.x * blockDim.x + threadIdx.x) * 8;
  if (c >= cols) return;
  const int64_t per = (rows + stripes - 1) / stripes;
  const int64_t r0 = (int64_t)blockIdx.y * per;
  const int64_t r1 = r0 + per < rows ? r0 + per : rows;
  float8 acc = {};
  for (int64_t r = r0; r < r1; ++r) {
    if (BF16) {
      const float8 v =
          load_bf16x8(reinterpret_cast<const unsigned short*>(dy) +
                      r * cols + c);
#pragma unroll
      for (int k = 0; k < 8; ++k) acc.v[k] += v.v[k];
    } else {
      const float* p = reinterpret_cast<const float*>(dy) + r * cols + c;
#pragma unroll
      for (int k = 0; k < 8; ++k) acc.v[k] += p[k];
    }
  }
  store_f32x8(partial + (int64_t)blockIdx.y * cols + c, acc);
}

template <bool BF16>
__global__ void colsum_reduce_kernel(void* __restrict__ db,
                                     const float* __restrict__ partial,
                                     int64_t stripes, int64_t cols) {
  const int64_t c = (int64_t)blockIdx.x * blockDim.x + threadIdx.x;
  if (c >= cols) return;
  float s = 0.f;
  for (int64_t p = 0; p < stripes; ++p) s += partial[p * cols + c];
  if (BF16)
    reinterpret_cast<unsigned short*>(db)[c] = f2bf(s);
  else
    reinterpret_cast<float*>(db)[c] = s;
}

template <bool DADD, bool COLSUM>
static void ln_bwd_fast_launch(void* dx, float* dgamma, float* dbeta,
                               float* colsum, const void* dy, const void* x,
                               const void* gamma, const void* dadd,
                               const float* mean, const float* rstd,
                               float* dg_part, float* db_part,
                               float* cs_part, int64_t rows, int64_t cols,
                               hipStream_t stream) {
  const int64_t wave_rows = (rows + 3) / 4;
  const int grid = (int)(wave_rows < 1024 ? wave_rows : 1024);
  if (cols <= 512)
    hipLaunchKernelGGL((layer_norm_bwd_bf16_kernel<1, true, DADD, COLSUM>),
                       dim3(grid), dim3(256), 0, stream, dx, dg_part,
                       db_part, cs_part, dy, x, gamma, dadd, mean, rstd,
                       rows, cols);
  else if (cols <= 1024)
    hipLaunchKernelGGL((layer_norm_bwd_bf16_kernel<2, true, DADD, COLSUM>),
                       dim3(grid), dim3(256), 0, stream, dx, dg_part,
                       db_part, cs_part, dy, x, gamma, dadd, mean, rstd,
                       rows, cols);
  else
    hipLaunchKernelGGL((layer_norm_bwd_bf16_kernel<4, false, DADD, COLSUM>),
                       dim3(grid), dim3(256), 0, stream, dx, dg_part,
                       db_part, cs_part, dy, x, gamma, dadd, mean, rstd,
                       rows, cols);
  hipLaunchKernelGGL(ln_bwd_partial_reduce_kernel<COLSUM>,
                     dim3((unsigned)((cols + 255) / 256), 64), dim3(256), 0,
                     stream, dgamma, dbeta, colsum, dg_part, db_part,
                     cs_part, (int64_t)grid * 4, cols);
}

extern "C" {

void epl_fused_adamw(float* master, unsigned short* param_bf16,
                     const void* grad, bool grad_bf16, float* m, float* v,
                     int64_t n, float lr, float beta1, float beta2, float eps,
                     float weight_decay, int step, float inv_scale,
                     hipStream_t stream) {
  const float inv_bias1 = inv_bias_correction(beta1, step);
  const float inv_bias2 = inv_bias_correction(beta2, step);
  const int grid = grid_for((n + 7) / 8);
  if (grad_bf16) {
    if (param_bf16)
      hipLaunchKernelGGL((fused_adamw_kernel<true, true>), dim3(grid),
                         dim3(kBlock), 0, stream, master, param_bf16, grad, m,
                         v, n, lr, beta1, beta2, eps, weight_decay, inv_bias1,
                         inv_bias2, inv_scale);
    else
      hipLaunchKernelGGL((fused_adamw_kernel<true, false>), dim3(grid),
                         dim3(kBlock), 0, stream, master, param_bf16, grad, m,
                         v, n, lr, beta1, beta2, eps, weight_decay, inv_bias1,
                         inv_bias2, inv_scale);
  } else {
    if (param_bf16)
      hipLaunchKernelGGL((fused_adamw_kernel<false, true>), dim3(grid),
                         dim3(kBlock), 0, stream, master, param_bf16, grad, m,
                         v, n, lr, beta1, beta2, eps, weight_decay, inv_bias1,
                         inv_bias2, inv_scale);
    else
      hipLaunchKernelGGL((fused_adamw_kernel<false, false>), dim3(grid),
                         dim3(kBlock), 0, stream, master, param_bf16, grad, m,
                         v, n, lr, beta1, beta2, eps, weight_decay, inv_bias1,
                         inv_bias2, inv_scale);
  }
}

void epl_lamb_phase1(const float* master, const void* grad, bool grad_bf16,
                     float* m, float* v, float* update, const int* chunk_of,
                     float* wnorm_sq, float* unorm_sq, int64_t n, float beta1,
                     float beta2, float eps, float weight_decay, int step,
                     float inv_scale, hipStream_t stream) {
  const float inv_bias1 = inv_bias_correction(beta1, step);
  const float inv_bias2 = inv_bias_correction(beta2, step);
  const int grid = grid_for(n);
  hipLaunchKernelGGL(lamb_phase1_kernel, dim3(grid), dim3(kBlock), 0, stream,
                     master, grad, grad_bf16, m, v, update, chunk_of, wnorm_sq,
                     unorm_sq, n, beta1, beta2, eps, weight_decay, inv_bias1,
                     inv_bias2, inv_scale);
}

void epl_lamb_phase2(float* master, unsigned short* param_bf16,
                     const float* update, const int* chunk_of,
                     const float* ratio, int64_t n, float lr,
                     hipStream_t stream) {
  const int grid = grid_for(n);
  hipLaunchKernelGGL(lamb_phase2_kernel, dim3(grid), dim3(kBlock), 0, stream,
                     master, param_bf16, update, chunk_of, ratio, n, lr);
}

static int ln_block_for(int64_t cols) {
  int64_t need = (cols + 7) / 8;
  if (need <= 64) return 64;
  if (need <= 128) return 128;
  if (need <= 192) return 192;
  return 256;
}

void epl_layer_norm_fwd(void* out, const void* x, const void* res,
                        void* sum_out, const void* gamma, const void* beta,
                        float* mean, float* rstd, int64_t rows, int64_t cols,
                        float eps, bool bf16, hipStream_t stream) {
  const int grid = (int)(rows < kMaxGrid ? rows : kMaxGrid);
  const bool has_res = res != nullptr;
  if (bf16 && cols % 8 == 0 && cols <= 2 * 256 * 8) {
    const int block = ln_block_for(cols);
    const bool two = cols > (int64_t)block * 8;
    if (has_res) {
      if (two)
        hipLaunchKernelGGL((layer_norm_fwd_bf16_kernel<true, 2>), dim3(grid),
                           dim3(block), 0, stream, out, x, res, sum_out,
                           gamma, beta, mean, rstd, rows, cols, eps);
      else
        hipLaunchKernelGGL((layer_norm_fwd_bf16_kernel<true, 1>), dim3(grid),
                           dim3(block), 0, stream, out, x, res, sum_out,
                           gamma, beta, mean, rstd, rows, cols, eps);
    } else {
      if (two)
        hipLaunchKernelGGL((layer_norm_fwd_bf16_kernel<false, 2>), dim3(grid),
                           dim3(block), 0, stream, out, x, res, sum_out,
                           gamma, beta, mean, rstd, rows, cols, eps);
      else
        hipLaunchKernelGGL((layer_norm_fwd_bf16_kernel<false, 1>), dim3(grid),
                           dim3(block), 0, stream, out, x, res, sum_out,
                           gamma, beta, mean, rstd, rows, cols, eps);
    }
    return;
  }
  if (bf16) {
    if (has_res)
      hipLaunchKernelGGL((layer_norm_fwd_kernel<true, true>), dim3(grid),
                         dim3(kBlock), 0, stream, out, x, res, sum_out,
                         gamma, beta, mean, rstd, rows, cols, eps);
    else
      hipLaunchKernelGGL((layer_norm_fwd_kernel<true, false>), dim3(grid),
                         dim3(kBlock), 0, stream, out, x, res, sum_out,
                         gamma, beta, mean, rstd, rows, cols, eps);
  } else {
    if (has_res)
      hipLaunchKernelGGL((layer_norm_fwd_kernel<false, true>), dim3(grid),
                         dim3(kBlock), 0, stream, out, x, res, sum_out,
                         gamma, beta, mean, rstd, rows, cols, eps);
    else
      hipLaunchKernelGGL((layer_norm_fwd_kernel<false, false>), dim3(grid),
                         dim3(kBlock), 0, stream, out, x, res, sum_out,
                         gamma, beta, mean, rstd, rows, cols, eps);
  }
}

void epl_layer_norm_bwd_fused(void* dx, float* dgamma, float* dbeta,
                              float* colsum, const void* dy, const void* x,
                              const void* gamma, const void* dadd,
                              const float* mean, const float* rstd,
                              float* dg_part, float* db_part,
                              float* cs_part, int64_t nparts, int64_t rows,
                              int64_t cols, bool bf16, hipStream_t stream) {
  if (bf16 && cols % 8 == 0 && cols <= 2048 && dg_part != nullptr) {
    const bool has_cs = colsum != nullptr && cs_part != nullptr;
    if (dadd != nullptr) {
      if (has_cs)
        ln_bwd_fast_launch<true, true>(dx, dgamma, dbeta, colsum, dy, x,
                                       gamma, dadd, mean, rstd, dg_part,
                                       db_part, cs_part, rows, cols, stream);
      else
        ln_bwd_fast_launch<true, false>(dx, dgamma, dbeta, colsum, dy, x,
                                        gamma, dadd, mean, rstd, dg_part,
                                        db_part, cs_part, rows, cols, stream);
    } else {
      if (has_cs)
        ln_bwd_fast_launch<false, true>(dx, dgamma, dbeta, colsum, dy, x,
                                        gamma, dadd, mean, rstd, dg_part,
                                        db_part, cs_part, rows, cols, stream);
      else
        ln_bwd_fast_launch<false, false>(dx, dgamma, dbeta, colsum, dy, x,
                                         gamma, dadd, mean, rstd, dg_part,
                                         db_part, cs_part, rows, cols,
                                         stream);
    }
    return;
  }
  int grid = (int)(rows < 1024 ? rows : 1024);
  const size_t lds_bytes = (size_t)cols * 2 * sizeof(float);
  if (bf16)
    hipLaunchKernelGGL((layer_norm_bwd_kernel<true>), dim3(grid),
                       dim3(kBlock), lds_bytes, stream, dx, dgamma, dbeta,
                       dy, x, gamma, mean, rstd, rows, cols);
  else
    hipLaunchKernelGGL((layer_norm_bwd_kernel<false>), dim3(grid),
                       dim3(kBlock), lds_bytes, stream, dx, dgamma, dbeta,
                       dy, x, gamma, mean, rstd, rows, cols);
}

void epl_layer_norm_bwd(void* dx, float* dgamma, float* dbeta, const void* dy,
                        const void* x, const void* gamma, const float* mean,
                        const float* rstd, float* dg_part, float* db_part,
                        int64_t nparts, int64_t rows, int64_t cols,
                        bool bf16, hipStream_t stream) {
  epl_layer_norm_bwd_fused(dx, dgamma, dbeta, nullptr, dy, x, gamma, nullptr,
                           mean, rstd, dg_part, db_part, nullptr, nparts,
                           rows, cols, bf16, stream);
}

void epl_bias_gelu_fwd(void* out, const void* x, const void* bias,
                       int64_t rows, int64_t cols, bool bf16,
                       hipStream_t stream) {
  int grid = grid_for((rows * cols + 7) / 8);
  if (bf16) {
    const int min_grid = (int)((cols / 8 + kBlock - 1) / kBlock);
    if (grid < min_grid) grid = min_grid;
    hipLaunchKernelGGL(bias_gelu_fwd_kernel<true>, dim3(grid), dim3(kBlock), 0,
                       stream, out, x, bias, rows, cols);
  } else
    hipLaunchKernelGGL(bias_gelu_fwd_kernel<false>, dim3(grid), dim3(kBlock),
                       0, stream, out, x, bias, rows, cols);
}

void epl_bias_gelu_bwd(void* dx, float* dbias, const void* dy, const void* x,
                       const void* bias, float* db_part, int64_t nwaves,
                       int64_t rows, int64_t cols, bool bf16,
                       hipStream_t stream) {
  if (bf16 && cols % 512 == 0 && db_part != nullptr) {
    const int grid = (int)(nwaves / 4);
    hipLaunchKernelGGL(bias_gelu_bwd_bf16_kernel, dim3(grid), dim3(256), 0,
                       stream, dx, db_part, dy, x, bias, rows, cols);
    const int64_t segs = cols / 512;
    hipLaunchKernelGGL(bias_gelu_db_reduce_kernel,
                       dim3((unsigned)((cols + 255) / 256), 32), dim3(256),
                       0, stream, dbias, db_part, nwaves, segs);
    return;
  }
  int grid = (int)(rows < 1024 ? rows : 1024);
  const size_t lds_bytes = (size_t)cols * sizeof(float);
  if (bf16)
    hipLaunchKernelGGL(bias_gelu_bwd_kernel<true>, dim3(grid), dim3(kBlock),
                       lds_bytes, stream, dx, dbias, dy, x, bias, rows,
                       cols);
  else
    hipLaunchKernelGGL(bias_gelu_bwd_kernel<false>, dim3(grid), dim3(kBlock),
                       lds_bytes, stream, dx, dbias, dy, x, bias, rows,
                       cols);
}

void epl_ce_rowstats(const void* logits, const int64_t* targets,
                     float* row_max, float* row_sumexp, float* target_logit,
                     int64_t rows, int64_t cols, int64_t vocab_begin,
                     int64_t ignore_index, bool bf16, hipStream_t stream) {
  const int grid = (int)(rows < kMaxGrid ? rows : kMaxGrid);
  if (bf16)
    hipLaunchKernelGGL(ce_rowstats_kernel<true>, dim3(grid), dim3(kBlock), 0,
                       stream, logits, targets, row_max, row_sumexp,
                       target_logit, rows, cols, vocab_begin, ignore_index);
  else
    hipLaunchKernelGGL(ce_rowstats_kernel<false>, dim3(grid), dim3(kBlock), 0,
                       stream, logits, targets, row_max, row_sumexp,
                       target_logit, rows, cols, vocab_begin, ignore_index);
}

void epl_ce_backward(void* dlogits, const void* logits, const int64_t* targets,
                     const float* gmax, const float* gsumexp,
                     const float* dloss, int64_t rows, int64_t cols,
                     int64_t vocab_begin, int64_t ignore_index, float scale,
                     bool bf16, hipStream_t stream) {
  const int grid = (int)(rows < kMaxGrid ? rows : kMaxGrid);
  if (bf16)
    hipLaunchKernelGGL(ce_backward_kernel<true>, dim3(grid), dim3(kBlock), 0,
                       stream, dlogits, logits, targets, gmax, gsumexp, dloss,
                       rows, cols, vocab_begin, ignore_index, scale);
  else
    hipLaunchKernelGGL(ce_backward_kernel<false>, dim3(grid), dim3(kBlock), 0,
                       stream, dlogits, logits, targets, gmax, gsumexp, dloss,
                       rows, cols, vocab_begin, ignore_index, scale);
}

void epl_scale(void* p, int64_t n, float s, bool bf16, hipStream_t stream) {
  const int grid = grid_for((n + 7) / 8);
  if (bf16)
    hipLaunchKernelGGL(scale_bf16_kernel, dim3(grid), dim3(kBlock), 0, stream,
                       reinterpret_cast<unsigned short*>(p), n, s);
  else
    hipLaunchKernelGGL(scale_f32_kernel, dim3(grid), dim3(kBlock), 0, stream,
                       reinterpret_cast<float*>(p), n, s);
}

void epl_f32_to_bf16(unsigned short* dst, const float* src, int64_t n,
                     hipStream_t stream) {
  const int grid = grid_for((n + 7) / 8);
  hipLaunchKernelGGL(f32_to_bf16_kernel, dim3(grid), dim3(kBlock), 0, stream,
                     dst, src, n);
}

void epl_bf16_to_f32(float* dst, const unsigned short* src, int64_t n,
                     hipStream_t stream) {
  const int grid = grid_for((n + 7) / 8);
  hipLaunchKernelGGL(bf16_to_f32_kernel, dim3(grid), dim3(kBlock), 0, stream,
                     dst, src, n);
}

void epl_sqnorm(const void* p, int64_t n, float* out, bool bf16,
                hipStream_t stream) {
  const int grid = grid_for(n) < 1024 ? grid_for(n) : 1024;
  if (bf16)
    hipLaunchKernelGGL(sqnorm_kernel<true>, dim3(grid), dim3(kBlock), 0,
                       stream, p, n, out);
  else
    hipLaunchKernelGGL(sqnorm_kernel<false>, dim3(grid), dim3(kBlock), 0,
                       stream, p, n, out);
}


void epl_colsum(void* db, const void* dy, float* partial, int64_t rows,
                int64_t cols, int64_t stripes, bool bf16,
                hipStream_t stream) {
  int64_t thr = cols / 8;
  thr = thr < 64 ? 64 : (thr > 256 ? 256 : thr);
  thr = (thr + 63) / 64 * 64;
  dim3 grid((unsigned)((cols / 8 + thr - 1) / thr), (unsigned)stripes);
  if (bf16)
    hipLaunchKernelGGL((colsum_partial_kernel<true>), grid, dim3((unsigned)thr),
                       0, stream, dy, partial, rows, cols, stripes);
  else
    hipLaunchKernelGGL((colsum_partial_kernel<false>), grid,
                       dim3((unsigned)thr), 0, stream, dy, partial, rows,
                       cols, stripes);
  dim3 rgrid((unsigned)((cols + 255) / 256));
  if (bf16)
    hipLaunchKernelGGL((colsum_reduce_kernel<true>), rgrid, dim3(256), 0,
                       stream, db, partial, stripes, cols);
  else
    hipLaunchKernelGGL((colsum_reduce_kernel<false>), rgrid, dim3(256), 0,
                       stream, db, partial, stripes, cols);
}

}
```

easyparallellibrary_amd/models/bert.py:

```python

import torch
import torch.nn as nn

import easyparallellibrary_amd as epl
from easyparallellibrary_amd.models.transformer import (Block, Embeddings,
                                                        LMHead, init_weights)

BERT_CONFIGS = {
    "bert-tiny": dict(layers=2, hidden=128, heads=2, ffn=512),
    "bert-base": dict(layers=12, hidden=768, heads=12, ffn=3072),
    "bert-large": dict(layers=24, hidden=1024, heads=16, ffn=4096),
}


class BertCore(nn.Module):

    def __init__(self, layers, hidden, heads, ffn, vocab_size, max_pos,
                 dropout=0.0, pad_token_id=None):
        super().__init__()
        self.pad_token_id = pad_token_id
        self.embeddings = Embeddings(vocab_size, hidden, max_pos)
        self.blocks = nn.ModuleList(
            Block(hidden, heads, ffn, causal=False, pre_ln=False,
                  dropout=dropout)
            for _ in range(layers))
        self.head = LMHead(hidden, vocab_size)

    def forward(self, ids, seqlens=None):
        if seqlens is None and self.pad_token_id is not None:
            seqlens = (ids != self.pad_token_id).sum(1).int()
        x = self.embeddings(ids)
        for b in self.blocks:
            x = b(x) if seqlens is None else b(x, seqlens=seqlens)
        return self.head(x)


class StagedModel(nn.Module):

    def __init__(self, stages):
        super().__init__()
        self.stages = nn.ModuleList(stages)

    def forward(self, x):
        for s in self.stages:
            x = s(x)
        return x


class _Stage(nn.Module):
    def __init__(self, mods):
        super().__init__()
        self.mods = nn.ModuleList(mods)

    def forward(self, x):
        for m in self.mods:
            x = m(x)
        return x


def build_bert(config="bert-large", vocab_size=30528, max_pos=512,
               num_stages=1, dropout=0.0, pad_token_id=None):
    cfg = BERT_CONFIGS[config] if isinstance(config, str) else dict(config)
    L, H, A, F = cfg["layers"], cfg["hidden"], cfg["heads"], cfg["ffn"]
    if num_stages <= 1:
        with epl.replicate(device_count=1, name="stage_0"):
            model = BertCore(L, H, A, F, vocab_size, max_pos,
                             dropout=dropout, pad_token_id=pad_token_id)
        return init_weights(model)
    if pad_token_id is not None:
        raise ValueError(
            "pad_token_id needs num_stages == 1: a pipeline stage boundary "
            "carries a single tensor (the hidden states), so the sequence "
            "lengths cannot reach the attention of the later stages")
    per = (L + num_stages - 1) // num_stages
    stages = []
    layer_idx = 0
    for s in range(num_stages):
        with epl.replicate(device_count=1, name="stage_{}".format(s)):
            mods = []
            if s == 0:
                mods.append(Embeddings(vocab_size, H, max_pos))
            n = min(per, L - layer_idx)
            mods.extend(Block(H, A, F, dropout=dropout)
                        for _ in range(n))
            layer_idx += n
            if s == num_stages - 1:
                mods.append(LMHead(H, vocab_size))
            stages.append(_Stage(mods))
    return init_weights(StagedModel(stages))


def synthetic_mlm_batch(batch, seq_len, vocab_size=30528, device="cpu",
                        mask_frac=0.15, seed=None, lengths=None,
                        pad_token_id=0):
    g = torch.Generator(device="cpu")
    if seed is not None:
        g.manual_seed(seed)
    ids = torch.randint(0, vocab_size, (batch, seq_len), generator=g)
    targets = ids.clone()
    mask = torch.rand(batch, seq_len, generator=g) < mask_frac
    targets[~mask] = -100
    ids[mask] = 103
    if lengths is not None:
        lens = torch.as_tensor(lengths, dtype=torch.long).reshape(batch, 1)
        pad = torch.arange(seq_len)[None, :] >= lens
        ids[pad] = pad_token_id
        targets[pad] = -100
    return ids.to(device), targets.to(device)
```

easyparallellibrary_amd/models/transformer.py:

```python

import os

import torch
import torch.nn as nn
import torch.nn.functional as F

_NATIVE_ATTN = os.environ.get("EPL_NATIVE_ATTENTION", "auto")

from easyparallellibrary_amd.ops.bias_gelu import FusedBiasGelu
from easyparallellibrary_amd.ops.bias_linear import FusedBiasLinear
from easyparallellibrary_amd.ops.layer_norm import (FusedLayerNorm,
                                                    linear_for_ln)

_FBG = os.environ.get("EPL_FUSED_BIAS_GRAD", "0") == "1"
_Linear = FusedBiasLinear if _FBG else nn.Linear

_QKV_SPLIT = os.environ.get("EPL_QKV_SPLIT", "1") == "1"


class _QKVSplit(torch.autograd.Function):

    @staticmethod
    def forward(ctx, qkv):
        q = qkv[:, :, 0].transpose(1, 2)
        k = qkv[:, :, 1].transpose(1, 2)
        v = qkv[:, :, 2].transpose(1, 2)
        return q, k, v

    @staticmethod
    def backward(ctx, dq, dk, dv):
        b, nh, s, d = dq.shape
        dqkv = torch.empty((b, s, 3, nh, d), dtype=dq.dtype,
                           device=dq.device)
        dqkv[:, :, 0].copy_(dq.transpose(1, 2))
        dqkv[:, :, 1].copy_(dk.transpose(1, 2))
        dqkv[:, :, 2].copy_(dv.transpose(1, 2))
        return dqkv


class SelfAttention(nn.Module):
    def __init__(self, hidden, num_heads, causal=False, dropout=0.0):
        super().__init__()
        assert hidden % num_heads == 0
        self.hidden = hidden
        self.num_heads = num_heads
        self.head_dim = hidden // num_heads
        self.causal = causal
        self.qkv = _Linear(hidden, 3 * hidden)
        self.proj = _Linear(hidden, hidden)
        self.dropout = dropout

    def forward(self, x, bias_grad_to_ln=False, seqlens=None):
        o = self._attend(x, seqlens)
        if bias_grad_to_ln:
            return linear_for_ln(self.proj, o)
        return self.proj(o)

    def _attend(self, x, seqlens=None):
        from easyparallellibrary_amd.ops.attention import (
            flash_attention, qkv_flash_attention, qkv_native_ok)
        b, s, h = x.shape
        qkv = self.qkv(x).reshape(b, s, 3, self.num_heads, self.head_dim)
        native_here = _NATIVE_ATTN in ("1", "auto")
        p = self.dropout if self.training else 0.0
        lens = {} if seqlens is None else {"seqlens": seqlens}
        if native_here and qkv_native_ok(qkv):
            o = qkv_flash_attention(qkv, causal=self.causal, dropout_p=p,
                                    **lens)
            return o.transpose(1, 2).reshape(b, s, h)
        if _QKV_SPLIT:
            q, k, v = _QKVSplit.apply(qkv)
        else:
            q, k, v = qkv.unbind(dim=2)
            q = q.transpose(1, 2)
            k = k.transpose(1, 2)
            v = v.transpose(1, 2)
        o = flash_attention(q, k, v, causal=self.causal,
                            allow_native=native_here, dropout_p=p, **lens)
        return o.transpose(1, 2).reshape(b, s, h)


class MLP(nn.Module):

    def __init__(self, hidden, ffn_hidden):
        super().__init__()
        self.fc1 = nn.Linear(hidden, ffn_hidden, bias=False)
        self.act = FusedBiasGelu(ffn_hidden)
        self.fc2 = _Linear(ffn_hidden, hidden)

    def forward(self, x, bias_grad_to_ln=False):
        h = self.act(self.fc1(x))
        if bias_grad_to_ln:
            return linear_for_ln(self.fc2, h)
        return self.fc2(h)


class Block(nn.Module):

    def __init__(self, hidden, num_heads, ffn_hidden, causal=False,
                 pre_ln=False, dropout=0.0):
        super().__init__()
        self.pre_ln = pre_ln
        self.ln1 = FusedLayerNorm(hidden)
        self.attn = SelfAttention(hidden, num_heads, causal=causal,
                                  dropout=dropout)
        self.ln2 = FusedLayerNorm(hidden)
        self.mlp = MLP(hidden, ffn_hidden)

    @staticmethod
    def _into_ln(mod, cls, x, **kwargs):
        kwargs = {k: v for k, v in kwargs.items() if v is not None}
        if type(mod) is cls:
            return mod(x, bias_grad_to_ln=True, **kwargs)
        return mod(x, **kwargs), None

    def forward(self, x, seqlens=None):
        if self.pre_ln:
            a, pb = self._into_ln(self.attn, SelfAttention, self.ln1(x),
                                  seqlens=seqlens)
            y, s = self.ln2.forward_with_sum(a, x, lin_bias=pb)
            return s + self.mlp(y)
        a, pb = self._into_ln(self.attn, SelfAttention, x, seqlens=seqlens)
        x = self.ln1(a, residual=x, lin_bias=pb)
        m, fb = self._into_ln(self.mlp, MLP, x)
        x = self.ln2(m, residual=x, lin_bias=fb)
        return x


class Embeddings(nn.Module):
    def __init__(self, vocab_size, hidden, max_positions, use_ln=True):
        super().__init__()
        self.tok = nn.Embedding(vocab_size, hidden)
        self.pos = nn.Embedding(max_positions, hidden)
        self.ln = FusedLayerNorm(hidden) if use_ln else None
        nn.init.normal_(self.tok.weight, std=0.02)
        nn.init.normal_(self.pos.weight, std=0.02)

    def forward(self, ids):
        s = ids.shape[1]
        pos = torch.arange(s, device=ids.device)
        x = self.tok(ids) + self.pos(pos)[None, :, :]
        if self.ln is not None:
            x = self.ln(x)
        return x


class LMHead(nn.Module):

    def __init__(self, hidden, vocab_size, use_ln=True):
        super().__init__()
        self.ln = FusedLayerNorm(hidden) if use_ln else None
        self.proj = nn.Linear(hidden, vocab_size, bias=False)
        nn.init.normal_(self.proj.weight, std=0.02)

    def forward(self, x):
        if self.ln is not None:
            x = self.ln(x)
        return self.proj(x)


def init_weights(model, std=0.02):
    for m in model.modules():
        if isinstance(m, nn.Linear):
            nn.init.normal_(m.weight, std=std)
            if m.bias is not None:
                nn.init.zeros_(m.bias)
    return model
```

easyparallellibrary_amd/ops/bias_gelu.py:

```python

import torch
import torch.nn as nn

from easyparallellibrary_amd.ops.dispatch import native_ext, use_native


def _gelu_tanh(x):
    return 0.5 * x * (1.0 + torch.tanh(
        0.7978845608028654 * (x + 0.044715 * x * x * x)))


class _FusedBiasGelu(torch.autograd.Function):
    @staticmethod
    def forward(ctx, x, bias):
        x = x.contiguous()
        cols = x.shape[-1]
        ctx.param_dtype = bias.dtype
        kbias = bias.contiguous().to(x.dtype)
        if use_native(x) and x.dtype in (torch.bfloat16, torch.float32) \
                and cols % 8 == 0:
            out = torch.empty_like(x)
            native_ext().bias_gelu_fwd(out, x, kbias)
        else:
            out = _gelu_tanh((x.float() + kbias.float())).to(x.dtype)
        ctx.save_for_backward(x, kbias)
        return out

    @staticmethod
    def backward(ctx, dy):
        x, bias = ctx.saved_tensors
        dy = dy.contiguous()
        cols = x.shape[-1]
        if use_native(x) and x.dtype in (torch.bfloat16, torch.float32) \
                and cols % 8 == 0:
            dx = torch.empty_like(x)
            dbias = torch.zeros(cols, dtype=torch.float32, device=x.device)
            native_ext().bias_gelu_bwd(dx, dbias, dy, x, bias)
        else:
            xb = x.float() + bias.float()
            t = torch.tanh(0.7978845608028654 * (xb + 0.044715 * xb ** 3))
            dgelu = 0.5 * (1 + t) + 0.5 * xb * (1 - t * t) * \
                0.7978845608028654 * (1 + 3 * 0.044715 * xb * xb)
            dx = (dy.float() * dgelu).to(x.dtype)
            dbias = dx.float().reshape(-1, cols).sum(dim=0)
        return dx, dbias.to(ctx.param_dtype)


class FusedBiasGelu(nn.Module):
    def __init__(self, hidden):
        super().__init__()
        self.bias = nn.Parameter(torch.zeros(hidden))

    def forward(self, x):
        return _FusedBiasGelu.apply(x, self.bias)
```

easyparallellibrary_amd/ops/distributed_losses.py:

```python

import torch

from easyparallellibrary_amd.ops.dispatch import native_ext, use_native


class _VocabParallelCE(torch.autograd.Function):
    @staticmethod
    def forward(ctx, logits, targets, comm, vocab_begin, ignore_index):
        rows = logits.shape[0]
        cols = logits.shape[1]
        dev = logits.device
        if use_native(logits):
            ext = native_ext()
            lmax = torch.empty(rows, dtype=torch.float32, device=dev)
            lsum = torch.empty(rows, dtype=torch.float32, device=dev)
            tlogit = torch.empty(rows, dtype=torch.float32, device=dev)
            ext.ce_rowstats(logits, targets, lmax, lsum, tlogit, vocab_begin,
                            ignore_index)
        else:
            lf = logits.float()
            lmax = lf.max(dim=1).values
            lsum = torch.exp(lf - lmax[:, None]).sum(dim=1)
            in_range = (targets != ignore_index) & (targets >= vocab_begin) \
                & (targets < vocab_begin + cols)
            safe = (targets - vocab_begin).clamp(0, cols - 1)
            tlogit = torch.where(
                in_range, lf.gather(1, safe[:, None]).squeeze(1),
                torch.zeros(rows, device=dev))
        if comm is not None and comm.size > 1:
            gmax = lmax.clone()
            comm.all_reduce(gmax, op="max")
            gsum = lsum * torch.exp(lmax - gmax)
            comm.all_reduce(gsum, op="sum")
            comm.all_reduce(tlogit, op="sum")
        else:
            gmax, gsum = lmax, lsum
        valid = (targets != ignore_index)
        losses = torch.where(
            valid, torch.log(gsum) + gmax - tlogit,
            torch.zeros_like(gmax))
        ctx.save_for_backward(logits, targets, gmax, gsum)
        ctx.comm = comm
        ctx.vocab_begin = vocab_begin
        ctx.ignore_index = ignore_index
        return losses

    @staticmethod
    def backward(ctx, dloss):
        logits, targets, gmax, gsum = ctx.saved_tensors
        dloss = dloss.contiguous().float()
        if use_native(logits):
            dlogits = torch.empty_like(logits)
            native_ext().ce_backward(dlogits, logits, targets, gmax, gsum,
                                     dloss, ctx.vocab_begin,
                                     ctx.ignore_index, 1.0)
        else:
            lf = logits.float()
            p = torch.exp(lf - gmax[:, None]) / gsum[:, None]
            cols = logits.shape[1]
            in_range = (targets != ctx.ignore_index) & \
                (targets >= ctx.vocab_begin) & \
                (targets < ctx.vocab_begin + cols)
            safe = (targets - ctx.vocab_begin).clamp(0, cols - 1)
            onehot = torch.zeros_like(p)
            onehot[in_range, safe[in_range]] = 1.0
            mask = (targets != ctx.ignore_index).float()[:, None]
            dlogits = ((p - onehot) * dloss[:, None] * mask).to(logits.dtype)
        return dlogits, None, None, None, None


def vocab_parallel_cross_entropy(logits, targets, comm=None, vocab_begin=0,
                                 ignore_index=-100):
    return _VocabParallelCE.apply(logits.contiguous(), targets.contiguous(),
                                  comm, vocab_begin, ignore_index)


class ParallelCrossEntropy(torch.nn.Module):

    def __init__(self, comm=None, vocab_begin=0, ignore_index=-100):
        super().__init__()
        self.comm = comm
        self.vocab_begin = vocab_begin
        self.ignore_index = ignore_index

    def forward(self, logits, targets):
        logits = logits.reshape(-1, logits.shape[-1])
        targets = targets.reshape(-1)
        losses = vocab_parallel_cross_entropy(
            logits, targets, self.comm, self.vocab_begin, self.ignore_index)
        valid = (targets != self.ignore_index).sum().clamp_min(1)
        return losses.sum() / valid
```

easyparallellibrary_amd/ops/layer_norm.py:

```python

import os

import torch
import torch.nn as nn
import torch.nn.functional as F

from easyparallellibrary_amd.ops.dispatch import native_ext, use_native


_LN_BWD_FUSE = os.environ.get("EPL_LN_BWD_FUSE", "1") == "1"


def _native_ok(x):
    return (use_native(x) and x.dtype in (torch.bfloat16, torch.float32)
            and x.shape[-1] % 8 == 0)


def _bwd_fast_ok(x):
    return (_native_ok(x) and x.dtype == torch.bfloat16
            and x.shape[-1] <= 2048)


def layer_norm_bwd_fused(dy, x, gamma, mean, rstd, dadd=None,
                         want_colsum=False):
    cols = x.shape[-1]
    dx = torch.empty_like(x)
    dgamma = torch.zeros(cols, dtype=torch.float32, device=x.device)
    dbeta = torch.zeros(cols, dtype=torch.float32, device=x.device)
    if _bwd_fast_ok(x):
        colsum = (torch.zeros(cols, dtype=torch.float32, device=x.device)
                  if want_colsum else None)
        if dadd is not None:
            dadd = dadd.contiguous().to(x.dtype)
        native_ext().layer_norm_bwd_fused(dx, dgamma, dbeta, dy, x, gamma,
                                          mean, rstd, dadd, colsum)
        return dx, dgamma, dbeta, colsum
    native_ext().layer_norm_bwd(dx, dgamma, dbeta, dy, x, gamma, mean, rstd)
    if dadd is not None:
        dx = dx + dadd
    colsum = (dx.reshape(-1, cols).sum(dim=0, dtype=torch.float32)
              if want_colsum else None)
    return dx, dgamma, dbeta, colsum


class _FusedLayerNorm(torch.autograd.Function):

    @staticmethod
    def forward(ctx, x, residual, gamma, beta, eps, lin_bias=None):
        x = x.contiguous()
        cols = x.shape[-1]
        rows = x.numel() // cols
        has_res = residual is not None
        if has_res:
            residual = residual.contiguous().to(x.dtype)
        ctx.param_dtype = gamma.dtype
        gamma = gamma.contiguous().to(x.dtype)
        beta = beta.contiguous().to(x.dtype)
        if _native_ok(x):
            mean = torch.empty(rows, dtype=torch.float32, device=x.device)
            rstd = torch.empty(rows, dtype=torch.float32, device=x.device)
            out = torch.empty_like(x)
            s = torch.empty_like(x) if has_res else None
            native_ext().layer_norm_fwd(out, x, residual, s, gamma,
                                        beta, mean, rstd, eps)
            norm_in = s if has_res else x
        else:
            norm_in = (x + residual) if has_res else x
            xf = norm_in.float().reshape(rows, cols)
            mu = xf.mean(dim=1)
            var = xf.var(dim=1, unbiased=False)
            rstd = (var + eps).rsqrt()
            mean = mu
            xhat = (xf - mu[:, None]) * rstd[:, None]
            out = (xhat * gamma.float() + beta.float()).to(x.dtype)
            out = out.reshape(x.shape)
            s = norm_in if has_res else None
        ctx.save_for_backward(norm_in, gamma, mean, rstd)
        ctx.has_res = has_res
        ctx.bias_dtype = lin_bias.dtype if lin_bias is not None else None
        ctx.fuse = _LN_BWD_FUSE
        if ctx.fuse:
            ctx.set_materialize_grads(False)
        if has_res:
            return out, s
        return out

    @staticmethod
    def backward(ctx, dy, *rest):
        norm_in, gamma, mean, rstd = ctx.saved_tensors
        ds = rest[0] if (ctx.has_res and rest) else None
        ds_late = None
        if not ctx.fuse:
            ds, ds_late = None, ds
        want_db = ctx.bias_dtype is not None and ctx.needs_input_grad[5]
        cols = norm_in.shape[-1]
        rows = norm_in.numel() // cols
        dgamma = dbeta = colsum = None
        if dy is None:
            dx = ds
            if dx is not None and want_db:
                colsum = dx.reshape(rows, cols).sum(dim=0,
                                                    dtype=torch.float32)
        elif _native_ok(norm_in):
            dx, dgamma, dbeta, colsum = layer_norm_bwd_fused(
                dy.contiguous(), norm_in, gamma.contiguous(), mean, rstd,
                dadd=ds, want_colsum=want_db)
        else:
            xf = norm_in.float().reshape(rows, cols)
            dyf = dy.float().reshape(rows, cols)
            xhat = (xf - mean[:, None]) * rstd[:, None]
            dyg = dyf * gamma.float()
            c1 = dyg.mean(dim=1, keepdim=True)
            c2 = (dyg * xhat).mean(dim=1, keepdim=True)
            dxf = (dyg - c1 - xhat * c2) * rstd[:, None]
            if ds is not None:
                dxf = dxf + ds.float().reshape(rows, cols)
            if want_db:
                colsum = dxf.sum(dim=0)
            dx = dxf.to(norm_in.dtype).reshape(norm_in.shape)
            dgamma = (dyf * xhat).sum(dim=0)
            dbeta = dyf.sum(dim=0)
        if dgamma is not None:
            dgamma = dgamma.to(ctx.param_dtype)
            dbeta = dbeta.to(ctx.param_dtype)
        if ds_late is not None:
            dx = dx + ds_late
        dbias = colsum.to(ctx.bias_dtype) if colsum is not None else None
        return (dx, dx if ctx.has_res else None, dgamma, dbeta, None, dbias)


class FusedLayerNorm(nn.Module):
    def __init__(self, hidden, eps=1e-5):
        super().__init__()
        self.weight = nn.Parameter(torch.ones(hidden))
        self.bias = nn.Parameter(torch.zeros(hidden))
        self.eps = eps

    def forward(self, x, residual=None, lin_bias=None):
        if residual is None:
            return _FusedLayerNorm.apply(x, None, self.weight, self.bias,
                                         self.eps, lin_bias)
        out, _ = _FusedLayerNorm.apply(x, residual, self.weight, self.bias,
                                       self.eps, lin_bias)
        return out

    def forward_with_sum(self, x, residual, lin_bias=None):
        return _FusedLayerNorm.apply(x, residual, self.weight, self.bias,
                                     self.eps, lin_bias)


def linear_for_ln(lin, x):
    if (_LN_BWD_FUSE and type(lin) is nn.Linear and lin.bias is not None
            and lin.bias.requires_grad and torch.is_grad_enabled()):
        return F.linear(x, lin.weight, lin.bias.detach()), lin.bias
    return lin(x), None
```

Baseline: 764.2 samples/s.

## Fork LayerNorm outputs to fuse gradient sum and emit typed param grads in-kernel

```diff
diff --git a/csrc/bindings.hip b/csrc/bindings.hip
--- a/csrc/bindings.hip
+++ b/csrc/bindings.hip
@@ -23,22 +23,24 @@
 void epl_layer_norm_fwd(void*, const void*, const void*, void*, const void*,
                         const void*, float*, float*, int64_t, int64_t, float,
                         bool, hipStream_t);
+int64_t epl_layer_norm_bwd_parts(int64_t);
 void epl_layer_norm_bwd(void*, float*, float*, const void*, const void*,
                         const void*, const float*, const float*, float*,
-                        float*, int64_t, int64_t, int64_t, bool,
-                        hipStream_t);
-void epl_layer_norm_bwd_fused(void*, float*, float*, float*, const void*,
+                        float*, int64_t, int64_t, bool, hipStream_t);
+void epl_layer_norm_bwd_fused(void*, void*, void*, void*, int, int, int,
                               const void*, const void*, const void*,
-                              const float*, const float*, float*, float*,
-                              float*, int64_t, int64_t, int64_t, bool,
-                              hipStream_t);
+                              const void*, const void*, const float*,
+                              const float*, float*, float*, float*, int64_t,
+                              int64_t, bool, hipStream_t);
 void epl_bias_gelu_fwd(void*, const void*, const void*, int64_t, int64_t,
                        bool, hipStream_t);
-void epl_bias_gelu_bwd(void*, float*, const void*, const void*, const void*,
-                       float*, int64_t, int64_t, int64_t, bool,
+int64_t epl_bias_gelu_bwd_parts(int64_t);
+void epl_bias_gelu_bwd(void*, void*, int, const void*, const void*,
+                       const void*, float*, int64_t, int64_t, bool,
                        hipStream_t);
 void epl_ce_rowstats(const void*, const int64_t*, float*, float*, float*,
-                     int64_t, int64_t, int64_t, int64_t, bool, hipStream_t);
+                     int64_t, int64_t, int64_t, int64_t, bool, bool,
+                     hipStream_t);
 void epl_ce_backward(void*, const void*, const int64_t*, const float*,
                      const float*, const float*, int64_t, int64_t, int64_t,
                      int64_t, float, bool, hipStream_t);
@@ -213,6 +215,14 @@
                      cols, (float)eps, bf16, cur_stream());
 }
 
+constexpr int kAccF32 = 0;
+
+int store_mode(const at::Tensor& t, const char* name) {
+  TORCH_CHECK(t.is_cuda(), name, " must be a device tensor");
+  TORCH_CHECK(t.is_contiguous(), name, " must be contiguous");
+  return is_bf16(t) ? 2 : 1;
+}
+
 void layer_norm_bwd(at::Tensor dx, at::Tensor dgamma, at::Tensor dbeta,
                     at::Tensor dy, at::Tensor x, at::Tensor gamma,
                     at::Tensor mean, at::Tensor rstd) {
@@ -228,10 +238,8 @@
   float* dbp = nullptr;
   at::Tensor ws;
   const bool fast = bf16 && cols % 8 == 0 && cols <= 2048;
-  int64_t nparts = 0;
   if (fast) {
-    const int64_t wave_rows = (rows + 3) / 4;
-    nparts = (wave_rows < 1024 ? wave_rows : 1024) * 4;
+    const int64_t nparts = epl_layer_norm_bwd_parts(rows);
     ws = at::empty({2, nparts, cols}, dgamma.options());
     dgp = ws.data_ptr<float>();
     dbp = dgp + nparts * cols;
@@ -239,61 +247,105 @@
   epl_layer_norm_bwd(dx.data_ptr(), dgamma.data_ptr<float>(),
                      dbeta.data_ptr<float>(), dy.data_ptr(), x.data_ptr(),
                      gamma.data_ptr(), mean.data_ptr<float>(),
-                     rstd.data_ptr<float>(), dgp, dbp, nparts, rows, cols,
-                     bf16, cur_stream());
-}
-
-void layer_norm_bwd_fused(at::Tensor dx, at::Tensor dgamma, at::Tensor dbeta,
-                          at::Tensor dy, at::Tensor x, at::Tensor gamma,
-                          at::Tensor mean, at::Tensor rstd,
-                          c10::optional<at::Tensor> dadd,
-                          c10::optional<at::Tensor> colsum_out) {
+                     rstd.data_ptr<float>(), dgp, dbp, rows, cols, bf16,
+                     cur_stream());
+}
+
+void ln_bwd_fused_impl(at::Tensor& dx, at::Tensor& dgamma, at::Tensor& dbeta,
+                       at::Tensor& dy, at::Tensor& x, at::Tensor& gamma,
+                       at::Tensor& mean, at::Tensor& rstd,
+                       c10::optional<at::Tensor>& dadd,
+                       c10::optional<at::Tensor>& colsum_out,
+                       c10::optional<at::Tensor>& dy2, bool accumulate,
+                       const char* who) {
   const bool bf16 = is_bf16(x);
   const int64_t cols = x.size(-1);
   const int64_t rows = x.numel() / cols;
   TORCH_CHECK(!bf16 || cols % 8 == 0, "bf16 LayerNorm needs cols % 8 == 0");
   TORCH_CHECK((size_t)cols * 2 * sizeof(float) <= 128 * 1024,
               "LayerNorm backward supports cols <= 16384");
-  check(dgamma, at::kFloat, "dgamma");
-  check(dbeta, at::kFloat, "dbeta");
+  int mode_g = kAccF32, mode_b = kAccF32, mode_c = kAccF32;
+  if (accumulate) {
+    check(dgamma, at::kFloat, "dgamma");
+    check(dbeta, at::kFloat, "dbeta");
+  } else {
+    mode_g = store_mode(dgamma, "dgamma");
+    mode_b = store_mode(dbeta, "dbeta");
+  }
+  check(dx, x.scalar_type(), "dx");
+  check(dy, x.scalar_type(), "dy");
+  check(x, x.scalar_type(), "x");
+  check(gamma, x.scalar_type(), "gamma");
+  check(mean, at::kFloat, "mean");
+  check(rstd, at::kFloat, "rstd");
   TORCH_CHECK(dx.numel() == x.numel() && dy.numel() == x.numel());
   TORCH_CHECK(dgamma.numel() == cols && dbeta.numel() == cols);
+  TORCH_CHECK(gamma.numel() == cols && mean.numel() == rows &&
+              rstd.numel() == rows);
   const bool fast = bf16 && cols % 8 == 0 && cols <= 2048;
-  const bool fused = dadd.has_value() || colsum_out.has_value();
-  TORCH_CHECK(fast || !fused,
-              "layer_norm_bwd_fused: dadd/colsum_out need the bf16 fast "
+  const bool fused =
+      dadd.has_value() || colsum_out.has_value() || dy2.has_value();
+  TORCH_CHECK(fast || (!fused && accumulate), who,
+              ": dadd / colsum_out / dy2 / typed outputs need the bf16 fast "
               "path (cols % 8 == 0, cols <= 2048)");
   const void* dadd_p = nullptr;
-  float* cs_out = nullptr;
+  const void* dy2_p = nullptr;
+  void* cs_out = nullptr;
   if (dadd.has_value()) {
     check(*dadd, x.scalar_type(), "dadd");
     TORCH_CHECK(dadd->numel() == x.numel(), "dadd shape mismatch");
     dadd_p = dadd->data_ptr();
   }
+  if (dy2.has_value()) {
+    check(*dy2, x.scalar_type(), "dy2");
+    TORCH_CHECK(dy2->numel() == x.numel(), "dy2 shape mismatch");
+    dy2_p = dy2->data_ptr();
+  }
   if (colsum_out.has_value()) {
-    check(*colsum_out, at::kFloat, "colsum_out");
+    if (accumulate)
+      check(*colsum_out, at::kFloat, "colsum_out");
+    else
+      mode_c = store_mode(*colsum_out, "colsum_out");
     TORCH_CHECK(colsum_out->numel() == cols, "colsum_out shape mismatch");
-    cs_out = colsum_out->data_ptr<float>();
+    cs_out = colsum_out->data_ptr();
   }
   float* dgp = nullptr;
   float* dbp = nullptr;
   float* csp = nullptr;
   at::Tensor ws;
-  int64_t nparts = 0;
   if (fast) {
-    const int64_t wave_rows = (rows + 3) / 4;
-    nparts = (wave_rows < 1024 ? wave_rows : 1024) * 4;
-    ws = at::empty({cs_out ? 3 : 2, nparts, cols}, dgamma.options());
+    const int64_t nparts = epl_layer_norm_bwd_parts(rows);
+    ws = at::empty({cs_out ? 3 : 2, nparts, cols},
+                   x.options().dtype(at::kFloat));
     dgp = ws.data_ptr<float>();
     dbp = dgp + nparts * cols;
     if (cs_out) csp = dbp + nparts * cols;
   }
-  epl_layer_norm_bwd_fused(dx.data_ptr(), dgamma.data_ptr<float>(),
-                           dbeta.data_ptr<float>(), cs_out, dy.data_ptr(),
-                           x.data_ptr(), gamma.data_ptr(), dadd_p,
+  epl_layer_norm_bwd_fused(dx.data_ptr(), dgamma.data_ptr(), dbeta.data_ptr(),
+                           cs_out, mode_g, mode_b, mode_c, dy.data_ptr(),
+                           dy2_p, x.data_ptr(), gamma.data_ptr(), dadd_p,
                            mean.data_ptr<float>(), rstd.data_ptr<float>(),
-                           dgp, dbp, csp, nparts, rows, cols, bf16,
-                           cur_stream());
+                           dgp, dbp, csp, rows, cols, bf16, cur_stream());
+}
+
+void layer_norm_bwd_fused(at::Tensor dx, at::Tensor dgamma, at::Tensor dbeta,
+                          at::Tensor dy, at::Tensor x, at::Tensor gamma,
+                          at::Tensor mean, at::Tensor rstd,
+                          c10::optional<at::Tensor> dadd,
+                          c10::optional<at::Tensor> colsum_out) {
+  c10::optional<at::Tensor> no_dy2;
+  ln_bwd_fused_impl(dx, dgamma, dbeta, dy, x, gamma, mean, rstd, dadd,
+                    colsum_out, no_dy2, true, "layer_norm_bwd_fused");
+}
+
+void layer_norm_bwd_typed(at::Tensor dx, at::Tensor dgamma, at::Tensor dbeta,
+                          at::Tensor dy, at::Tensor x, at::Tensor gamma,
+                          at::Tensor mean, at::Tensor rstd,
+                          c10::optional<at::Tensor> dadd,
+                          c10::optional<at::Tensor> colsum_out,
+                          c10::optional<at::Tensor> dy2) {
+  ln_bwd_fused_impl(dx, dgamma, dbeta, dy, x, gamma, mean, rstd, dadd,
+                    colsum_out, dy2, false, "layer_norm_bwd_typed");
 }
 
 void bias_gelu_fwd(at::Tensor out, at::Tensor x, at::Tensor bias) {
@@ -305,34 +357,55 @@
                     bf16, cur_stream());
 }
 
-void bias_gelu_bwd(at::Tensor dx, at::Tensor dbias, at::Tensor dy,
-                   at::Tensor x, at::Tensor bias) {
+void bias_gelu_bwd_impl(at::Tensor& dx, at::Tensor& dbias, at::Tensor& dy,
+                        at::Tensor& x, at::Tensor& bias, bool accumulate) {
   const bool bf16 = is_bf16(x);
   const int64_t cols = x.size(-1);
   const int64_t rows = x.numel() / cols;
   TORCH_CHECK(!bf16 || cols % 8 == 0, "bf16 bias_gelu needs cols % 8 == 0");
   TORCH_CHECK((size_t)cols * sizeof(float) <= 128 * 1024,
               "bias_gelu backward supports cols <= 32768");
-  check(dbias, at::kFloat, "dbias");
+  const bool fast = bf16 && cols % 512 == 0;
+  int mode = kAccF32;
+  if (accumulate) {
+    check(dbias, at::kFloat, "dbias");
+  } else {
+    TORCH_CHECK(fast, "bias_gelu_bwd_typed needs the bf16 fast path "
+                      "(cols % 512 == 0)");
+    mode = store_mode(dbias, "dbias");
+  }
+  check(dx, x.scalar_type(), "dx");
+  check(dy, x.scalar_type(), "dy");
+  check(x, x.scalar_type(), "x");
+  check(bias, x.scalar_type(), "bias");
+  TORCH_CHECK(dx.numel() == x.numel() && dy.numel() == x.numel());
+  TORCH_CHECK(dbias.numel() == cols && bias.numel() == cols);
   float* dbp = nullptr;
-  int64_t nwaves = 0;
   at::Tensor ws;
-  if (bf16 && cols % 512 == 0) {
-    const int64_t segs = cols / 512;
-    int64_t per_seg = rows < 1024 ? rows : 1024;
-    per_seg = (per_seg + 3) / 4 * 4;
-    nwaves = segs * per_seg;
-    ws = at::empty({nwaves, 512}, dbias.options());
+  if (fast) {
+    ws = at::empty({epl_bias_gelu_bwd_parts(rows), cols},
+                   x.options().dtype(at::kFloat));
     dbp = ws.data_ptr<float>();
   }
-  epl_bias_gelu_bwd(dx.data_ptr(), dbias.data_ptr<float>(), dy.data_ptr(),
-                    x.data_ptr(), bias.data_ptr(), dbp, nwaves, rows, cols,
-                    bf16, cur_stream());
+  epl_bias_gelu_bwd(dx.data_ptr(), dbias.data_ptr(), mode, dy.data_ptr(),
+                    x.data_ptr(), bias.data_ptr(), dbp, rows, cols, bf16,
+                    cur_stream());
+}
+
+void bias_gelu_bwd(at::Tensor dx, at::Tensor dbias, at::Tensor dy,
+                   at::Tensor x, at::Tensor bias) {
+  bias_gelu_bwd_impl(dx, dbias, dy, x, bias, true);
+}
+
+void bias_gelu_bwd_typed(at::Tensor dx, at::Tensor dbias, at::Tensor dy,
+                         at::Tensor x, at::Tensor bias) {
+  bias_gelu_bwd_impl(dx, dbias, dy, x, bias, false);
 }
 
 void ce_rowstats(at::Tensor logits, at::Tensor targets, at::Tensor row_max,
                  at::Tensor row_sumexp, at::Tensor target_logit,
-                 int64_t vocab_begin, int64_t ignore_index) {
+                 int64_t vocab_begin, int64_t ignore_index,
+                 bool skip_ignored) {
   const bool bf16 = is_bf16(logits);
   const int64_t cols = logits.size(-1);
   const int64_t rows = logits.numel() / cols;
@@ -340,7 +413,7 @@
   epl_ce_rowstats(logits.data_ptr(), targets.data_ptr<int64_t>(),
                   row_max.data_ptr<float>(), row_sumexp.data_ptr<float>(),
                   target_logit.data_ptr<float>(), rows, cols, vocab_begin,
-                  ignore_index, bf16, cur_stream());
+                  ignore_index, skip_ignored, bf16, cur_stream());
 }
 
 void ce_backward(at::Tensor dlogits, at::Tensor logits, at::Tensor targets,
@@ -864,9 +937,18 @@
         py::arg("dgamma"), py::arg("dbeta"), py::arg("dy"), py::arg("x"),
         py::arg("gamma"), py::arg("mean"), py::arg("rstd"),
         py::arg("dadd") = py::none(), py::arg("colsum_out") = py::none());
+  m.def("layer_norm_bwd_typed", &layer_norm_bwd_typed, py::arg("dx"),
+        py::arg("dgamma"), py::arg("dbeta"), py::arg("dy"), py::arg("x"),
+        py::arg("gamma"), py::arg("mean"), py::arg("rstd"),
+        py::arg("dadd") = py::none(), py::arg("colsum_out") = py::none(),
+        py::arg("dy2") = py::none());
   m.def("bias_gelu_fwd", &bias_gelu_fwd);
   m.def("bias_gelu_bwd", &bias_gelu_bwd);
-  m.def("ce_rowstats", &ce_rowstats);
+  m.def("bias_gelu_bwd_typed", &bias_gelu_bwd_typed);
+  m.def("ce_rowstats", &ce_rowstats, py::arg("logits"), py::arg("targets"),
+        py::arg("row_max"), py::arg("row_sumexp"), py::arg("target_logit"),
+        py::arg("vocab_begin"), py::arg("ignore_index"),
+        py::arg("skip_ignored") = false);
   m.def("ce_backward", &ce_backward);
   m.def("scale_", &scale_);
   m.def("f32_to_bf16", &f32_to_bf16);
diff --git a/csrc/kernels/kernels.hip b/csrc/kernels/kernels.hip
--- a/csrc/kernels/kernels.hip
+++ b/csrc/kernels/kernels.hip
@@ -348,21 +348,22 @@
   }
 }
 
-template <int CHUNKS, bool CACHE, bool DADD, bool COLSUM>
+template <int CHUNKS, bool CACHE, bool DADD, bool COLSUM, bool DY2>
 __global__ __launch_bounds__(256, CHUNKS == 1 ? 5 : 3) void
 layer_norm_bwd_bf16_kernel(
     void* __restrict__ dx, float* __restrict__ dg_part,
     float* __restrict__ db_part, float* __restrict__ cs_part,
-    const void* __restrict__ dy, const void* __restrict__ x,
+    const void* __restrict__ dy, const void* __restrict__ dy2,
+    const void* __restrict__ x,
     const void* __restrict__ gamma, const void* __restrict__ dadd,
     const float* __restrict__ mean_in, const float* __restrict__ rstd_in,
     int64_t rows, int64_t cols) {
   using T = unsigned short;
   const int lane = threadIdx.x & 63;
-  const int wid = threadIdx.x >> 6;
+  const int wid = __builtin_amdgcn_readfirstlane(threadIdx.x >> 6);
   const int wpb = blockDim.x >> 6;
   constexpr bool FUSED = DADD || COLSUM;
-  constexpr bool G_LDS = FUSED && CHUNKS == 4;
+  constexpr bool G_LDS = (FUSED || DY2) && CHUNKS == 4;
   constexpr bool G_PK = FUSED && CHUNKS == 1;
   constexpr bool G_F32 = !G_LDS && !G_PK;
   __shared__ __attribute__((aligned(16))) T g_lds[G_LDS ? CHUNKS * 512 : 8];
@@ -415,6 +416,12 @@
       const int64_t c = ((int64_t)lane + k * 64) * 8;
       if (c >= cols) continue;
       float8 d = load_bf16x8(reinterpret_cast<const T*>(dy) + base + c);
+      if (DY2) {
+        const float8 d2 =
+            load_bf16x8(reinterpret_cast<const T*>(dy2) + base + c);
+#pragma unroll
+        for (int j = 0; j < 8; ++j) d.v[j] += d2.v[j];
+      }
       float8 f = load_bf16x8(reinterpret_cast<const T*>(x) + base + c);
       const float8 g = gamma_at(k, c);
 #pragma unroll
@@ -447,6 +454,12 @@
         xh = c_xhat[k];
       } else {
         float8 d = load_bf16x8(reinterpret_cast<const T*>(dy) + base + c);
+        if (DY2) {
+          const float8 d2 =
+              load_bf16x8(reinterpret_cast<const T*>(dy2) + base + c);
+#pragma unroll
+          for (int j = 0; j < 8; ++j) d.v[j] += d2.v[j];
+        }
         float8 f = load_bf16x8(reinterpret_cast<const T*>(x) + base + c);
 #pragma unroll
         for (int j = 0; j < 8; ++j) {
@@ -476,34 +489,103 @@
       store_bf16x8(reinterpret_cast<T*>(dx) + base + c, o);
     }
   }
-  const int64_t prow = ((int64_t)blockIdx.x * wpb + wid) * cols;
-#pragma unroll
-  for (int k = 0; k < CHUNKS; ++k) {
-    const int64_t c = ((int64_t)lane + k * 64) * 8;
-    if (c >= cols) continue;
-    store_f32x8(dg_part + prow + c, acc_dg[k]);
-    store_f32x8(db_part + prow + c, acc_db[k]);
-    if (COLSUM) store_f32x8(cs_part + prow + c, acc_cs[k]);
-  }
-}
-
-template <bool COLSUM>
-__global__ void ln_bwd_partial_reduce_kernel(
-    float* __restrict__ dgamma, float* __restrict__ dbeta,
-    float* __restrict__ colsum, const float* __restrict__ dg_part,
-    const float* __restrict__ db_part, const float* __restrict__ cs_part,
-    int64_t nparts, int64_t cols) {
-  const int64_t c = (int64_t)blockIdx.x * blockDim.x + threadIdx.x;
-  if (c >= cols) return;
-  float sg = 0.f, sb = 0.f, sc = 0.f;
-  for (int64_t p = blockIdx.y; p < nparts; p += gridDim.y) {
-    sg += dg_part[p * cols + c];
-    sb += db_part[p * cols + c];
-    if (COLSUM) sc += cs_part[p * cols + c];
-  }
-  atomicAdd(&dgamma[c], sg);
-  atomicAdd(&dbeta[c], sb);
-  if (COLSUM) atomicAdd(&colsum[c], sc);
+  constexpr int PLANES = COLSUM ? 3 : 2;
+  constexpr int GROUP = CHUNKS <= 2 ? PLANES : 1;
+  __shared__ __attribute__((aligned(16))) float red[3][GROUP][CHUNKS * 512];
+  const int64_t prow = (int64_t)blockIdx.x * cols;
+  auto post = [&](const float8 (&acc)[CHUNKS], int slot) {
+    if (wid == 0) return;
+#pragma unroll
+    for (int k = 0; k < CHUNKS; ++k) {
+      const int c = (lane + k * 64) * 8;
+      if (c < cols) store_f32x8(&red[wid - 1][slot][c], acc[k]);
+    }
+  };
+  auto fold = [&](float8 (&acc)[CHUNKS], int slot, float* part) {
+    if (wid != 0) return;
+#pragma unroll
+    for (int k = 0; k < CHUNKS; ++k) {
+      const int c = (lane + k * 64) * 8;
+      if (c >= cols) continue;
+      for (int w = 0; w < 3; ++w) {
+        const float8 o = load_f32x8(&red[w][slot][c]);
+#pragma unroll
+        for (int j = 0; j < 8; ++j) acc[k].v[j] += o.v[j];
+      }
+      store_f32x8(part + prow + c, acc[k]);
+    }
+  };
+  if constexpr (GROUP > 1) {
+    post(acc_dg, 0);
+    post(acc_db, 1);
+    if constexpr (COLSUM) post(acc_cs, GROUP - 1);
+    __syncthreads();
+    fold(acc_dg, 0, dg_part);
+    fold(acc_db, 1, db_part);
+    if constexpr (COLSUM) fold(acc_cs, GROUP - 1, cs_part);
+  } else {
+    post(acc_dg, 0);
+    __syncthreads();
+    fold(acc_dg, 0, dg_part);
+    __syncthreads();
+    post(acc_db, 0);
+    __syncthreads();
+    fold(acc_db, 0, db_part);
+    if constexpr (COLSUM) {
+      __syncthreads();
+      post(acc_cs, 0);
+      __syncthreads();
+      fold(acc_cs, 0, cs_part);
+    }
+  }
+}
+
+enum : int { kRedAccF32 = 0, kRedStoreF32 = 1, kRedStoreBF16 = 2 };
+
+struct RedPlane {
+  void* out;
+  const float* part;
+  int mode;
+};
+struct RedPlanes {
+  RedPlane p[3];
+};
+
+constexpr int kRedCols = 16, kRedSlices = 64, kRedDepth = 16;
+
+__global__ __launch_bounds__(kRedCols * kRedSlices) void
+partial_rows_reduce_kernel(RedPlanes planes, int64_t nparts, int64_t cols) {
+  __shared__ float lds[kRedSlices][kRedCols];
+  const RedPlane pl = planes.p[blockIdx.y];
+  const int cx = threadIdx.x % kRedCols;
+  const int sy = threadIdx.x / kRedCols;
+  const int64_t c = (int64_t)blockIdx.x * kRedCols + cx;
+  float sum = 0.f;
+  if (c < cols) {
+    for (int64_t p0 = sy; p0 < nparts; p0 += kRedSlices * kRedDepth) {
+      float v[kRedDepth];
+#pragma unroll
+      for (int i = 0; i < kRedDepth; ++i) {
+        const int64_t p = p0 + (int64_t)i * kRedSlices;
+        v[i] = p < nparts ? pl.part[p * cols + c] : 0.f;
+      }
+#pragma unroll
+      for (int i = 0; i < kRedDepth; ++i) sum += v[i];
+    }
+  }
+  lds[sy][cx] = sum;
+  __syncthreads();
+  if (sy == 0 && c < cols) {
+    float t = lds[0][cx];
+#pragma unroll
+    for (int i = 1; i < kRedSlices; ++i) t += lds[i][cx];
+    if (pl.mode == kRedStoreBF16)
+      reinterpret_cast<unsigned short*>(pl.out)[c] = f2bf(t);
+    else if (pl.mode == kRedStoreF32)
+      reinterpret_cast<float*>(pl.out)[c] = t;
+    else
+      reinterpret_cast<float*>(pl.out)[c] += t;
+  }
 }
 
 template <bool BF16>
@@ -654,7 +736,6 @@
   const int wid = threadIdx.x >> 6;
   const int wpb = blockDim.x >> 6;
   const int64_t segs = cols / 512;
-  const int64_t total = rows * segs;
   float8 acc;
 #pragma unroll
   for (int j = 0; j < 8; ++j) acc.v[j] = 0.f;
@@ -662,8 +743,9 @@
   const int64_t nwaves = (int64_t)gridDim.x * wpb;
   const int64_t myseg = wave_id % segs;
   const int64_t c0 = myseg * 512 + (int64_t)lane * 8;
+  const int64_t step = nwaves / segs;
   float8 bw = load_bf16x8(reinterpret_cast<const T*>(bias) + c0);
-  for (int64_t row = wave_id / segs; row < rows; row += nwaves / segs) {
+  for (int64_t row = wave_id / segs; row < rows; row += step) {
     const int64_t base = row * cols + c0;
     float8 d = load_bf16x8(reinterpret_cast<const T*>(dy) + base);
     float8 f = load_bf16x8(reinterpret_cast<const T*>(x) + base);
@@ -677,21 +759,6 @@
     store_bf16x8_pk(reinterpret_cast<T*>(dx) + base, o);
   }
   store_f32x8(db_part + wave_id * 512 + (int64_t)lane * 8, acc);
-}
-
-__global__ void bias_gelu_db_reduce_kernel(
-    float* __restrict__ dbias, const float* __restrict__ db_part,
-    int64_t nwaves, int64_t segs) {
-  const int64_t c = (int64_t)blockIdx.x * blockDim.x + threadIdx.x;
-  if (c >= segs * 512) return;
-  const int64_t seg = c / 512;
-  const int64_t off = c % 512;
-  float sum = 0.f;
-  for (int64_t p = seg + blockIdx.y * segs; p < nwaves;
-       p += (int64_t)gridDim.y * segs) {
-    sum += db_part[p * 512 + off];
-  }
-  atomicAdd(&dbias[c], sum);
 }
 
 template <bool BF16>
@@ -744,12 +811,21 @@
                                    float* __restrict__ row_sumexp,
                                    float* __restrict__ target_logit,
                                    int64_t rows, int64_t cols,
-                                   int64_t vocab_begin, int64_t ignore_index) {
+                                   int64_t vocab_begin, int64_t ignore_index,
+                                   bool skip_ignored) {
   __shared__ float lds[8];
   using T = unsigned short;
   const bool vec = BF16 && (cols % 8 == 0);
   for (int64_t row = blockIdx.x; row < rows; row += gridDim.x) {
     const int64_t base = row * cols;
+    if (skip_ignored && targets[row] == ignore_index) {
+      if (threadIdx.x == 0) {
+        row_max[row] = 0.f;
+        row_sumexp[row] = 1.f;
+        target_logit[row] = 0.f;
+      }
+      continue;
+    }
     float vmax = -INFINITY;
     if (vec) {
       const T* lr = reinterpret_cast<const T*>(logits) + base;
@@ -818,10 +894,26 @@
   const bool vec = BF16 && (cols % 8 == 0);
   for (int64_t row = blockIdx.x; row < rows; row += gridDim.x) {
     const int64_t base = row * cols;
+    const int64_t tgt = targets[row];
+    if (tgt == ignore_index) {
+      if (vec) {
+        T* dr = reinterpret_cast<T*>(dlogits) + base;
+        for (int64_t c = threadIdx.x * 8; c < cols;
+             c += (int64_t)blockDim.x * 8)
+          *reinterpret_cast<uint4*>(dr + c) = make_uint4(0u, 0u, 0u, 0u);
+      } else {
+        for (int64_t c = threadIdx.x; c < cols; c += blockDim.x) {
+          if (BF16)
+            reinterpret_cast<T*>(dlogits)[base + c] = 0;
+          else
+            reinterpret_cast<float*>(dlogits)[base + c] = 0.f;
+        }
+      }
+      continue;
+    }
     const float m = gmax[row];
     const float inv_sum = 1.f / gsumexp[row];
-    const int64_t tgt = targets[row];
-    const float dl = (tgt == ignore_index ? 0.f : dloss[row] * scale);
+    const float dl = dloss[row] * scale;
     const int64_t tc = tgt - vocab_begin;
     if (vec) {
       const T* lr = reinterpret_cast<const T*>(logits) + base;
@@ -967,35 +1059,53 @@
     reinterpret_cast<float*>(db)[c] = s;
 }
 
+inline int64_t ln_bwd_parts(int64_t rows) {
+  const int64_t wave_rows = (rows + 3) / 4;
+  return wave_rows < 1024 ? (wave_rows > 0 ? wave_rows : 1) : 1024;
+}
+
+struct LnBwdArgs {
+  void* dx;
+  RedPlanes outs;
+  const void *dy, *dy2, *x, *gamma, *dadd;
+  const float *mean, *rstd;
+  int64_t rows, cols;
+  hipStream_t stream;
+};
+
+template <bool DADD, bool COLSUM, bool DY2>
+static void ln_bwd_fast_launch(const LnBwdArgs& a) {
+  const int grid = (int)ln_bwd_parts(a.rows);
+  float* dg_part = const_cast<float*>(a.outs.p[0].part);
+  float* db_part = const_cast<float*>(a.outs.p[1].part);
+  float* cs_part = const_cast<float*>(a.outs.p[2].part);
+  if (a.cols <= 512)
+    hipLaunchKernelGGL(
+        (layer_norm_bwd_bf16_kernel<1, true, DADD, COLSUM, DY2>), dim3(grid),
+        dim3(256), 0, a.stream, a.dx, dg_part, db_part, cs_part, a.dy, a.dy2,
+        a.x, a.gamma, a.dadd, a.mean, a.rstd, a.rows, a.cols);
+  else if (a.cols <= 1024)
+    hipLaunchKernelGGL(
+        (layer_norm_bwd_bf16_kernel<2, true, DADD, COLSUM, DY2>), dim3(grid),
+        dim3(256), 0, a.stream, a.dx, dg_part, db_part, cs_part, a.dy, a.dy2,
+        a.x, a.gamma, a.dadd, a.mean, a.rstd, a.rows, a.cols);
+  else
+    hipLaunchKernelGGL(
+        (layer_norm_bwd_bf16_kernel<4, false, DADD, COLSUM, DY2>), dim3(grid),
+        dim3(256), 0, a.stream, a.dx, dg_part, db_part, cs_part, a.dy, a.dy2,
+        a.x, a.gamma, a.dadd, a.mean, a.rstd, a.rows, a.cols);
+  hipLaunchKernelGGL(partial_rows_reduce_kernel,
+                     dim3((unsigned)((a.cols + kRedCols - 1) / kRedCols),
+                          COLSUM ? 3 : 2),
+                     dim3(kRedCols * kRedSlices), 0, a.stream, a.outs, (int64_t)grid, a.cols);
+}
+
 template <bool DADD, bool COLSUM>
-static void ln_bwd_fast_launch(void* dx, float* dgamma, float* dbeta,
-                               float* colsum, const void* dy, const void* x,
-                               const void* gamma, const void* dadd,
-                               const float* mean, const float* rstd,
-                               float* dg_part, float* db_part,
-                               float* cs_part, int64_t rows, int64_t cols,
-                               hipStream_t stream) {
-  const int64_t wave_rows = (rows + 3) / 4;
-  const int grid = (int)(wave_rows < 1024 ? wave_rows : 1024);
-  if (cols <= 512)
-    hipLaunchKernelGGL((layer_norm_bwd_bf16_kernel<1, true, DADD, COLSUM>),
-                       dim3(grid), dim3(256), 0, stream, dx, dg_part,
-                       db_part, cs_part, dy, x, gamma, dadd, mean, rstd,
-                       rows, cols);
-  else if (cols <= 1024)
-    hipLaunchKernelGGL((layer_norm_bwd_bf16_kernel<2, true, DADD, COLSUM>),
-                       dim3(grid), dim3(256), 0, stream, dx, dg_part,
-                       db_part, cs_part, dy, x, gamma, dadd, mean, rstd,
-                       rows, cols);
+static void ln_bwd_fast_dy2(const LnBwdArgs& a) {
+  if (a.dy2 != nullptr)
+    ln_bwd_fast_launch<DADD, COLSUM, true>(a);
   else
-    hipLaunchKernelGGL((layer_norm_bwd_bf16_kernel<4, false, DADD, COLSUM>),
-                       dim3(grid), dim3(256), 0, stream, dx, dg_part,
-                       db_part, cs_part, dy, x, gamma, dadd, mean, rstd,
-                       rows, cols);
-  hipLaunchKernelGGL(ln_bwd_partial_reduce_kernel<COLSUM>,
-                     dim3((unsigned)((cols + 255) / 256), 64), dim3(256), 0,
-                     stream, dgamma, dbeta, colsum, dg_part, db_part,
-                     cs_part, (int64_t)grid * 4, cols);
+    ln_bwd_fast_launch<DADD, COLSUM, false>(a);
 }
 
 extern "C" {
@@ -1115,56 +1225,58 @@
   }
 }
 
-void epl_layer_norm_bwd_fused(void* dx, float* dgamma, float* dbeta,
-                              float* colsum, const void* dy, const void* x,
-                              const void* gamma, const void* dadd,
-                              const float* mean, const float* rstd,
-                              float* dg_part, float* db_part,
-                              float* cs_part, int64_t nparts, int64_t rows,
+int64_t epl_layer_norm_bwd_parts(int64_t rows) { return ln_bwd_parts(rows); }
+
+void epl_layer_norm_bwd_fused(void* dx, void* dgamma, void* dbeta,
+                              void* colsum, int mode_g, int mode_b,
+                              int mode_c, const void* dy, const void* dy2,
+                              const void* x, const void* gamma,
+                              const void* dadd, const float* mean,
+                              const float* rstd, float* dg_part,
+                              float* db_part, float* cs_part, int64_t rows,
                               int64_t cols, bool bf16, hipStream_t stream) {
   if (bf16 && cols % 8 == 0 && cols <= 2048 && dg_part != nullptr) {
     const bool has_cs = colsum != nullptr && cs_part != nullptr;
+    LnBwdArgs a;
+    a.dx = dx;
+    a.outs.p[0] = {dgamma, dg_part, mode_g};
+    a.outs.p[1] = {dbeta, db_part, mode_b};
+    a.outs.p[2] = {has_cs ? colsum : nullptr, has_cs ? cs_part : nullptr,
+                   mode_c};
+    a.dy = dy; a.dy2 = dy2; a.x = x; a.gamma = gamma; a.dadd = dadd;
+    a.mean = mean; a.rstd = rstd;
+    a.rows = rows; a.cols = cols; a.stream = stream;
     if (dadd != nullptr) {
-      if (has_cs)
-        ln_bwd_fast_launch<true, true>(dx, dgamma, dbeta, colsum, dy, x,
-                                       gamma, dadd, mean, rstd, dg_part,
-                                       db_part, cs_part, rows, cols, stream);
-      else
-        ln_bwd_fast_launch<true, false>(dx, dgamma, dbeta, colsum, dy, x,
-                                        gamma, dadd, mean, rstd, dg_part,
-                                        db_part, cs_part, rows, cols, stream);
+      if (has_cs) ln_bwd_fast_dy2<true, true>(a);
+      else ln_bwd_fast_dy2<true, false>(a);
     } else {
-      if (has_cs)
-        ln_bwd_fast_launch<false, true>(dx, dgamma, dbeta, colsum, dy, x,
-                                        gamma, dadd, mean, rstd, dg_part,
-                                        db_part, cs_part, rows, cols, stream);
-      else
-        ln_bwd_fast_launch<false, false>(dx, dgamma, dbeta, colsum, dy, x,
-                                         gamma, dadd, mean, rstd, dg_part,
-                                         db_part, cs_part, rows, cols,
-                                         stream);
+      if (has_cs) ln_bwd_fast_dy2<false, true>(a);
+      else ln_bwd_fast_dy2<false, false>(a);
     }
     return;
   }
   int grid = (int)(rows < 1024 ? rows : 1024);
   const size_t lds_bytes = (size_t)cols * 2 * sizeof(float);
+  float* dg = reinterpret_cast<float*>(dgamma);
+  float* db = reinterpret_cast<float*>(dbeta);
   if (bf16)
     hipLaunchKernelGGL((layer_norm_bwd_kernel<true>), dim3(grid),
-                       dim3(kBlock), lds_bytes, stream, dx, dgamma, dbeta,
+                       dim3(kBlock), lds_bytes, stream, dx, dg, db,
                        dy, x, gamma, mean, rstd, rows, cols);
   else
     hipLaunchKernelGGL((layer_norm_bwd_kernel<false>), dim3(grid),
-                       dim3(kBlock), lds_bytes, stream, dx, dgamma, dbeta,
+                       dim3(kBlock), lds_bytes, stream, dx, dg, db,
                        dy, x, gamma, mean, rstd, rows, cols);
 }
 
 void epl_layer_norm_bwd(void* dx, float* dgamma, float* dbeta, const void* dy,
                         const void* x, const void* gamma, const float* mean,
                         const float* rstd, float* dg_part, float* db_part,
-                        int64_t nparts, int64_t rows, int64_t cols,
-                        bool bf16, hipStream_t stream) {
-  epl_layer_norm_bwd_fused(dx, dgamma, dbeta, nullptr, dy, x, gamma, nullptr,
-                           mean, rstd, dg_part, db_part, nullptr, nparts,
+                        int64_t rows, int64_t cols, bool bf16,
+                        hipStream_t stream) {
+  epl_layer_norm_bwd_fused(dx, dgamma, dbeta, nullptr, kRedAccF32,
+                           kRedAccF32, kRedAccF32, dy, nullptr, x, gamma,
+                           nullptr, mean, rstd, dg_part, db_part, nullptr,
                            rows, cols, bf16, stream);
 }
 
@@ -1182,45 +1294,57 @@
                        0, stream, out, x, bias, rows, cols);
 }
 
-void epl_bias_gelu_bwd(void* dx, float* dbias, const void* dy, const void* x,
-                       const void* bias, float* db_part, int64_t nwaves,
+int64_t epl_bias_gelu_bwd_parts(int64_t rows) {
+  int64_t per_seg = rows < 1024 ? (rows > 0 ? rows : 1) : 1024;
+  return (per_seg + 3) / 4 * 4;
+}
+
+void epl_bias_gelu_bwd(void* dx, void* dbias, int mode, const void* dy,
+                       const void* x, const void* bias, float* db_part,
                        int64_t rows, int64_t cols, bool bf16,
                        hipStream_t stream) {
   if (bf16 && cols % 512 == 0 && db_part != nullptr) {
-    const int grid = (int)(nwaves / 4);
+    const int64_t segs = cols / 512;
+    const int64_t per_seg = epl_bias_gelu_bwd_parts(rows);
+    const int grid = (int)(segs * per_seg / 4);
     hipLaunchKernelGGL(bias_gelu_bwd_bf16_kernel, dim3(grid), dim3(256), 0,
                        stream, dx, db_part, dy, x, bias, rows, cols);
-    const int64_t segs = cols / 512;
-    hipLaunchKernelGGL(bias_gelu_db_reduce_kernel,
-                       dim3((unsigned)((cols + 255) / 256), 32), dim3(256),
-                       0, stream, dbias, db_part, nwaves, segs);
+    RedPlanes outs;
+    outs.p[0] = {dbias, db_part, mode};
+    outs.p[1] = outs.p[2] = {nullptr, nullptr, mode};
+    hipLaunchKernelGGL(partial_rows_reduce_kernel,
+                       dim3((unsigned)((cols + kRedCols - 1) / kRedCols), 1),
+                       dim3(kRedCols * kRedSlices), 0,
+                       stream, outs, per_seg, cols);
     return;
   }
   int grid = (int)(rows < 1024 ? rows : 1024);
   const size_t lds_bytes = (size_t)cols * sizeof(float);
+  float* db = reinterpret_cast<float*>(dbias);
   if (bf16)
     hipLaunchKernelGGL(bias_gelu_bwd_kernel<true>, dim3(grid), dim3(kBlock),
-                       lds_bytes, stream, dx, dbias, dy, x, bias, rows,
-                       cols);
+                       lds_bytes, stream, dx, db, dy, x, bias, rows, cols);
   else
     hipLaunchKernelGGL(bias_gelu_bwd_kernel<false>, dim3(grid), dim3(kBlock),
-                       lds_bytes, stream, dx, dbias, dy, x, bias, rows,
-                       cols);
+                       lds_bytes, stream, dx, db, dy, x, bias, rows, cols);
 }
 
 void epl_ce_rowstats(const void* logits, const int64_t* targets,
                      float* row_max, float* row_sumexp, float* target_logit,
                      int64_t rows, int64_t cols, int64_t vocab_begin,
-                     int64_t ignore_index, bool bf16, hipStream_t stream) {
+                     int64_t ignore_index, bool skip_ignored, bool bf16,
+                     hipStream_t stream) {
   const int grid = (int)(rows < kMaxGrid ? rows : kMaxGrid);
   if (bf16)
     hipLaunchKernelGGL(ce_rowstats_kernel<true>, dim3(grid), dim3(kBlock), 0,
                        stream, logits, targets, row_max, row_sumexp,
-                       target_logit, rows, cols, vocab_begin, ignore_index);
+                       target_logit, rows, cols, vocab_begin, ignore_index,
+                       skip_ignored);
   else
     hipLaunchKernelGGL(ce_rowstats_kernel<false>, dim3(grid), dim3(kBlock), 0,
                        stream, logits, targets, row_max, row_sumexp,
-                       target_logit, rows, cols, vocab_begin, ignore_index);
+                       target_logit, rows, cols, vocab_begin, ignore_index,
+                       skip_ignored);
 }
 
 void epl_ce_backward(void* dlogits, const void* logits, const int64_t* targets,
diff --git a/easyparallellibrary_amd/models/bert.py b/easyparallellibrary_amd/models/bert.py
--- a/easyparallellibrary_amd/models/bert.py
+++ b/easyparallellibrary_amd/models/bert.py
@@ -29,9 +29,20 @@
     def forward(self, ids, seqlens=None):
         if seqlens is None and self.pad_token_id is not None:
             seqlens = (ids != self.pad_token_id).sum(1).int()
-        x = self.embeddings(ids)
-        for b in self.blocks:
-            x = b(x) if seqlens is None else b(x, seqlens=seqlens)
+        n = len(self.blocks)
+        plain = [type(b) is Block and not b.pre_ln for b in self.blocks]
+        if n and plain[0] and type(self.embeddings) is Embeddings:
+            x, x_res = self.embeddings(ids, pair_out=True)
+        else:
+            x = x_res = self.embeddings(ids)
+        for i, b in enumerate(self.blocks):
+            if plain[i]:
+                pair_out = i + 1 < n and plain[i + 1]
+                x = b(x, seqlens=seqlens, x_res=x_res, pair_out=pair_out)
+                x, x_res = x if pair_out else (x, x)
+            else:
+                x = b(x) if seqlens is None else b(x, seqlens=seqlens)
+                x_res = x
         return self.head(x)
 
 
diff --git a/easyparallellibrary_amd/models/transformer.py b/easyparallellibrary_amd/models/transformer.py
--- a/easyparallellibrary_amd/models/transformer.py
+++ b/easyparallellibrary_amd/models/transformer.py
@@ -114,17 +114,22 @@
             return mod(x, bias_grad_to_ln=True, **kwargs)
         return mod(x, **kwargs), None
 
-    def forward(self, x, seqlens=None):
+    def forward(self, x, seqlens=None, x_res=None, pair_out=False):
+        if x_res is None:
+            x_res = x
         if self.pre_ln:
+            if pair_out or x_res is not x:
+                raise ValueError("x_res / pair_out are post-LN only")
             a, pb = self._into_ln(self.attn, SelfAttention, self.ln1(x),
                                   seqlens=seqlens)
             y, s = self.ln2.forward_with_sum(a, x, lin_bias=pb)
             return s + self.mlp(y)
         a, pb = self._into_ln(self.attn, SelfAttention, x, seqlens=seqlens)
-        x = self.ln1(a, residual=x, lin_bias=pb)
-        m, fb = self._into_ln(self.mlp, MLP, x)
-        x = self.ln2(m, residual=x, lin_bias=fb)
-        return x
+        h, h_res = self.ln1.forward_pair(a, residual=x_res, lin_bias=pb)
+        m, fb = self._into_ln(self.mlp, MLP, h)
+        if pair_out:
+            return self.ln2.forward_pair(m, residual=h_res, lin_bias=fb)
+        return self.ln2(m, residual=h_res, lin_bias=fb)
 
 
 class Embeddings(nn.Module):
@@ -136,10 +141,12 @@
         nn.init.normal_(self.tok.weight, std=0.02)
         nn.init.normal_(self.pos.weight, std=0.02)
 
-    def forward(self, ids):
+    def forward(self, ids, pair_out=False):
         s = ids.shape[1]
         pos = torch.arange(s, device=ids.device)
         x = self.tok(ids) + self.pos(pos)[None, :, :]
+        if pair_out:
+            return self.ln.forward_pair(x) if self.ln is not None else (x, x)
         if self.ln is not None:
             x = self.ln(x)
         return x
diff --git a/easyparallellibrary_amd/ops/bias_gelu.py b/easyparallellibrary_amd/ops/bias_gelu.py
--- a/easyparallellibrary_amd/ops/bias_gelu.py
+++ b/easyparallellibrary_amd/ops/bias_gelu.py
@@ -31,6 +31,13 @@
         x, bias = ctx.saved_tensors
         dy = dy.contiguous()
         cols = x.shape[-1]
+        if use_native(x) and x.dtype == torch.bfloat16 and cols % 512 == 0 \
+                and ctx.param_dtype in (torch.bfloat16, torch.float32):
+            dx = torch.empty_like(x)
+            dbias = torch.empty(cols, dtype=ctx.param_dtype,
+                                device=x.device)
+            native_ext().bias_gelu_bwd_typed(dx, dbias, dy, x, bias)
+            return dx, dbias
         if use_native(x) and x.dtype in (torch.bfloat16, torch.float32) \
                 and cols % 8 == 0:
             dx = torch.empty_like(x)
diff --git a/easyparallellibrary_amd/ops/distributed_losses.py b/easyparallellibrary_amd/ops/distributed_losses.py
--- a/easyparallellibrary_amd/ops/distributed_losses.py
+++ b/easyparallellibrary_amd/ops/distributed_losses.py
@@ -16,7 +16,7 @@
             lsum = torch.empty(rows, dtype=torch.float32, device=dev)
             tlogit = torch.empty(rows, dtype=torch.float32, device=dev)
             ext.ce_rowstats(logits, targets, lmax, lsum, tlogit, vocab_begin,
-                            ignore_index)
+                            ignore_index, skip_ignored=True)
         else:
             lf = logits.float()
             lmax = lf.max(dim=1).values
@@ -64,8 +64,9 @@
             safe = (targets - ctx.vocab_begin).clamp(0, cols - 1)
             onehot = torch.zeros_like(p)
             onehot[in_range, safe[in_range]] = 1.0
-            mask = (targets != ctx.ignore_index).float()[:, None]
-            dlogits = ((p - onehot) * dloss[:, None] * mask).to(logits.dtype)
+            valid = (targets != ctx.ignore_index)[:, None]
+            dlogits = torch.where(valid, (p - onehot) * dloss[:, None],
+                                  torch.zeros_like(p)).to(logits.dtype)
         return dlogits, None, None, None, None
 
 
diff --git a/easyparallellibrary_amd/ops/layer_norm.py b/easyparallellibrary_amd/ops/layer_norm.py
--- a/easyparallellibrary_amd/ops/layer_norm.py
+++ b/easyparallellibrary_amd/ops/layer_norm.py
@@ -9,6 +9,8 @@
 
 
 _LN_BWD_FUSE = os.environ.get("EPL_LN_BWD_FUSE", "1") == "1"
+
+_LN_BWD_FORK = os.environ.get("EPL_LN_BWD_FORK", "1") == "1"
 
 
 def _native_ok(x):
@@ -22,31 +24,46 @@
 
 
 def layer_norm_bwd_fused(dy, x, gamma, mean, rstd, dadd=None,
-                         want_colsum=False):
+                         want_colsum=False, dy2=None, param_dtype=None,
+                         colsum_dtype=None):
     cols = x.shape[-1]
+    param_dtype = param_dtype or torch.float32
+    colsum_dtype = colsum_dtype or torch.float32
     dx = torch.empty_like(x)
-    dgamma = torch.zeros(cols, dtype=torch.float32, device=x.device)
-    dbeta = torch.zeros(cols, dtype=torch.float32, device=x.device)
     if _bwd_fast_ok(x):
-        colsum = (torch.zeros(cols, dtype=torch.float32, device=x.device)
+        typed = (torch.bfloat16, torch.float32)
+        pd = param_dtype if param_dtype in typed else torch.float32
+        cd = colsum_dtype if colsum_dtype in typed else torch.float32
+        dgamma = torch.empty(cols, dtype=pd, device=x.device)
+        dbeta = torch.empty(cols, dtype=pd, device=x.device)
+        colsum = (torch.empty(cols, dtype=cd, device=x.device)
                   if want_colsum else None)
         if dadd is not None:
             dadd = dadd.contiguous().to(x.dtype)
-        native_ext().layer_norm_bwd_fused(dx, dgamma, dbeta, dy, x, gamma,
-                                          mean, rstd, dadd, colsum)
-        return dx, dgamma, dbeta, colsum
+        if dy2 is not None:
+            dy2 = dy2.contiguous().to(x.dtype)
+        native_ext().layer_norm_bwd_typed(dx, dgamma, dbeta, dy, x, gamma,
+                                          mean, rstd, dadd, colsum, dy2)
+        if colsum is not None:
+            colsum = colsum.to(colsum_dtype)
+        return (dx, dgamma.to(param_dtype), dbeta.to(param_dtype), colsum)
+    if dy2 is not None:
+        dy = dy + dy2
+    dgamma = torch.zeros(cols, dtype=torch.float32, device=x.device)
+    dbeta = torch.zeros(cols, dtype=torch.float32, device=x.device)
     native_ext().layer_norm_bwd(dx, dgamma, dbeta, dy, x, gamma, mean, rstd)
     if dadd is not None:
         dx = dx + dadd
     colsum = (dx.reshape(-1, cols).sum(dim=0, dtype=torch.float32)
-              if want_colsum else None)
-    return dx, dgamma, dbeta, colsum
+              .to(colsum_dtype) if want_colsum else None)
+    return dx, dgamma.to(param_dtype), dbeta.to(param_dtype), colsum
 
 
 class _FusedLayerNorm(torch.autograd.Function):
 
     @staticmethod
-    def forward(ctx, x, residual, gamma, beta, eps, lin_bias=None):
+    def forward(ctx, x, residual, gamma, beta, eps, lin_bias=None,
+                fork=False):
         x = x.contiguous()
         cols = x.shape[-1]
         rows = x.numel() // cols
@@ -81,13 +98,20 @@
         ctx.fuse = _LN_BWD_FUSE
         if ctx.fuse:
             ctx.set_materialize_grads(False)
+        ctx.fork = fork
+        outs = (out, out.view_as(out)) if fork else (out,)
         if has_res:
-            return out, s
-        return out
+            outs = outs + (s,)
+        return outs if len(outs) > 1 else out
 
     @staticmethod
     def backward(ctx, dy, *rest):
         norm_in, gamma, mean, rstd = ctx.saved_tensors
+        dy2 = None
+        if ctx.fork:
+            dy2, rest = rest[0], rest[1:]
+            if dy is None:
+                dy, dy2 = dy2, None
         ds = rest[0] if (ctx.has_res and rest) else None
         ds_late = None
         if not ctx.fuse:
@@ -104,8 +128,11 @@
         elif _native_ok(norm_in):
             dx, dgamma, dbeta, colsum = layer_norm_bwd_fused(
                 dy.contiguous(), norm_in, gamma.contiguous(), mean, rstd,
-                dadd=ds, want_colsum=want_db)
+                dadd=ds, want_colsum=want_db, dy2=dy2,
+                param_dtype=ctx.param_dtype, colsum_dtype=ctx.bias_dtype)
         else:
+            if dy2 is not None:
+                dy = dy + dy2
             xf = norm_in.float().reshape(rows, cols)
             dyf = dy.float().reshape(rows, cols)
             xhat = (xf - mean[:, None]) * rstd[:, None]
@@ -126,7 +153,8 @@
         if ds_late is not None:
             dx = dx + ds_late
         dbias = colsum.to(ctx.bias_dtype) if colsum is not None else None
-        return (dx, dx if ctx.has_res else None, dgamma, dbeta, None, dbias)
+        return (dx, dx if ctx.has_res else None, dgamma, dbeta, None, dbias,
+                None)
 
 
 class FusedLayerNorm(nn.Module):
@@ -144,6 +172,14 @@
                                        self.eps, lin_bias)
         return out
 
+    def forward_pair(self, x, residual=None, lin_bias=None):
+        if not (_LN_BWD_FORK and torch.is_grad_enabled()):
+            y = self.forward(x, residual=residual, lin_bias=lin_bias)
+            return y, y
+        outs = _FusedLayerNorm.apply(x, residual, self.weight, self.bias,
+                                     self.eps, lin_bias, True)
+        return outs[0], outs[1]
+
     def forward_with_sum(self, x, residual, lin_bias=None):
         return _FusedLayerNorm.apply(x, residual, self.weight, self.bias,
                                      self.eps, lin_bias)
```

After: 785.4 samples/s (median of 6 runs). 2.8% higher.
